# NikNazarov/TorchPIV

Measured on AMD Instinct MI355X. Metric: image-pairs/sec at 4 MP, wind=64 ov=32 2-pass CWS; % HBM roofline, higher is better.
Workload: dtype u32 exact sums + f64 / f32

## Files before the change

torchpiv_amd/csrc/piv_kernels.h:

```cpp
#pragma once
#include <hip/hip_runtime.h>
#include <stdint.h>

namespace tpiv {

enum { MODE_PASS1 = 0, MODE_DWS = 1, MODE_CWS = 2, MODE_CWSF = 3 };

struct PassParams {
    const uint8_t* A;
    const uint8_t* B;
    int batch, H, W;
    int ws, ov, n_rows, n_cols;
    const double* u0;
    const double* v0;
    const double* u2;
    const double* v2;
    const uint8_t* pmask;
    double* u;
    double* v;
    uint8_t* val;
    double* du;
    double* dv;
    double val_ratio;
    int val_win;
    int precision;
    float* dbg_win;
    float* dbg_corr;
    unsigned long long* stamps;
    float* peak_raw;
    unsigned* work_ctr;
    int* slow_list;
    unsigned* slow_count;
    int list_mode;
    uint4* cand;
    int* fb_list;
    unsigned* fb_count;
    float exact_band;
    float exact_band_range;
    hipEvent_t* sub_events;
    unsigned groups_magic, ncols_magic;
    int groups_shift, ncols_shift;
};

constexpr double EXACT_ETA = 6.66;
enum { EXACT_FFT_RADIX2 = 0, EXACT_FFT_MIXED = 1, EXACT_FFT_PLAIN = 2 };
inline double exact_gamma_u(int ws, int kind) {
    double lg = 0.0, rt = 1.0;
    for (int n = 1; n < ws; n *= 2) lg += 1.0;
    while ((rt + 1.0) * (rt + 1.0) <= (double)ws) rt += 1.0;
    rt += 1.0;
    const double f1 = kind == EXACT_FFT_PLAIN ? (ws + 3) * rt : (kind == EXACT_FFT_MIXED ? 64.0 : lg * EXACT_ETA);
    const double i1 = kind == EXACT_FFT_PLAIN ? (double)(ws + 3) : f1;
    return 2.0 * (2.0 * f1 + 1.0) + 5.0 + 2.0 * i1;
}
inline float exact_band_coef(int ws, int kind = EXACT_FFT_RADIX2) {
    return (float)(2.0 * exact_gamma_u(ws, kind) * (1.0 + 1.0 / 16) * 5.9604644775390625e-08);
}
constexpr int EXACT_MAX_SECOND = 3, EXACT_MAX_MIN = 4;

struct PredictParams {
    int batch, mode;
    int nrc, ncc, nrf, ncf;
    const double* Ay;
    const double* Ax;
    const double* u_c;
    const double* v_c;
    const uint8_t* val_c;
    double* T;
    double* u0;
    double* v0;
    double* u2;
    double* v2;
};

struct BandedPredictParams {
    int batch, mode;
    int nrc, ncc, nrf, ncf;
    int KY, KX;
    int nrfp;
    const double* Wy32;
    const int* k0y32;
    const double* Ax32;
    const int* k0x32;
    const double* u_c;
    const double* v_c;
    const uint8_t* val_c;
    double* T1;
    double* u0;
    double* v0;
    double* u2;
    double* v2;
    uint8_t* mask_out;
};

struct PostvalParams {
    double* u;
    double* v;
    const uint8_t* invalid;
    uint8_t* cls;
    int* counts;
    int batch, n_rows, n_cols;
};
hipError_t launch_postval(const PostvalParams& p, hipStream_t stream);
hipError_t launch_postval_compact(const double* u, const double* v, const uint8_t* cls, const int* counts, int batch, int n_rows,
                                  int n_cols, int* offsets, int* ring_rc, double* ring_uv, int* hole_rc, hipStream_t stream);
hipError_t launch_finish_fields(const double* u, const double* v, int batch, int n_rows, int n_cols, double scale, double dt,
                                double* fu, double* fv, hipStream_t stream);
hipError_t launch_ensemble_moments(const double* U, const double* V, int n, long long cells, double* out, hipStream_t stream);

hipError_t launch_bmp_unpack(const uint8_t* raw, const long long* desc, const uint8_t* lut, int n_files, int H, int W,
                             uint8_t* out, hipStream_t stream);

hipError_t launch_xcorr(const PassParams& p, int mode, int n_cu, hipStream_t stream);
constexpr size_t TILE_CTR_BYTES = 8 * 16 * sizeof(unsigned), TILE_SLOW_HDR_BYTES = 256;
#ifndef TPIV_SPLIT64
#define TPIV_SPLIT64 1
#endif
constexpr bool tile_split64(int ws, int mode) { return TPIV_SPLIT64 && ws == 64 && mode == MODE_CWS; }
#ifndef TPIV_OCC64C
#define TPIV_OCC64C 2
#endif
constexpr int tile_occ_c(int ws, int mode) {
    return (ws != 8 && ws != 16 && ws != 32 && ws != 64) ? 0
           : (ws == 16 ? 4 : ((ws == 32 || (ws == 64 && (mode != MODE_CWS || TPIV_OCC64C == 3))) ? 3 : 2));
}
inline int tile_occ(int ws, int mode) { return tile_occ_c(ws, mode); }
#ifdef __HIPCC__
template <int MODE>
__device__ __forceinline__ void pred_half_shift(const PassParams& p, size_t i, double& sx, double& sy) {
    const bool compact = p.pmask != nullptr;
    const double* __restrict__ us = compact ? p.u0 : p.u2;
    const double* __restrict__ vs = compact ? p.v0 : p.v2;
    double u = us[i], v = vs[i];
    if constexpr (MODE == MODE_DWS) {
        const uint8_t* mp = compact ? p.pmask + i : reinterpret_cast<const uint8_t*>(us + i);
        const bool zero = *mp != 0 && compact;
        const double uz = zero ? 0.0 : u, vz = zero ? 0.0 : v;
        sx = compact ? rint(uz / 2) : u;
        sy = compact ? rint(vz / 2) : v;
    } else {
        sx = compact ? u / 2 : u;
        sy = compact ? v / 2 : v;
    }
}
__device__ __forceinline__ void pred_half_shift_cws_f32(const PassParams& p, size_t i, float& vx, float& vy) {
    const bool compact = p.pmask != nullptr;
    const double* __restrict__ us = compact ? p.u0 : p.u2;
    const double* __restrict__ vs = compact ? p.v0 : p.v2;
    const float k = compact ? 0.5f : 1.0f;
    vx = (float)us[i] * k;
    vy = (float)vs[i] * k;
}
__device__ __forceinline__ void pred_fallback(const PassParams& p, size_t i, double& u0, double& v0) {
    const bool compact = p.pmask != nullptr;
    const uint8_t* mp = compact ? p.pmask + i : reinterpret_cast<const uint8_t*>(p.u0 + i);
    const bool zero = *mp != 0 && compact;
    u0 = zero ? 0.0 : p.u0[i];
    v0 = zero ? 0.0 : p.v0[i];
}
#endif

const char* xcorr_kernel_name(int ws, int mode, int precision, char* buf, int len);
size_t peak_raw_bytes(int ws, int batch, int n_windows, int precision, bool force_generic = false);
bool exact_refine_size(int ws);
size_t exact_fallback_count_offset(int batch, int n_windows);
hipError_t launch_peaks_from_maps(const PassParams& p, const float* maps, int n_maps, int planar, hipStream_t stream);
hipError_t launch_predict_mfma(const BandedPredictParams& q, hipStream_t stream);
hipError_t launch_predict(const PredictParams& q, hipStream_t stream);

}
```

torchpiv_amd/csrc/piv_launch.hip:

```cpp
#include <hip/hip_runtime.h>
#include <stdint.h>
#include <stdio.h>
#include <stdlib.h>

#include "piv_kernels.h"

namespace tpiv {

hipError_t launch_xcorr_ws8(const PassParams& p, int mode, int n_cu, hipStream_t stream);
hipError_t launch_xcorr_w8(const PassParams& p, int mode, int n_cu, hipStream_t stream);
hipError_t launch_peak_debug_w8(const PassParams& p, const float* maps, int n_maps, hipStream_t stream);
hipError_t launch_xcorr_ws16(const PassParams& p, int mode, int n_cu, hipStream_t stream);
hipError_t launch_xcorr_ws32(const PassParams& p, int mode, int n_cu, hipStream_t stream);
hipError_t launch_xcorr_ws64(const PassParams& p, int mode, int n_cu, hipStream_t stream);
hipError_t launch_xcorr_big128_pass1(const PassParams& p, int n_cu, hipStream_t stream);
hipError_t launch_peak_debug_ws8(const PassParams& p, const float* maps, int n_maps, int planar, hipStream_t stream);
hipError_t launch_peak_debug_ws16(const PassParams& p, const float* maps, int n_maps, int planar, hipStream_t stream);
hipError_t launch_peak_debug_ws32(const PassParams& p, const float* maps, int n_maps, int planar, hipStream_t stream);
hipError_t launch_peak_debug_ws64(const PassParams& p, const float* maps, int n_maps, int planar, hipStream_t stream);
hipError_t launch_peak_debug_ws128(const PassParams& p, const float* maps, int n_maps, hipStream_t stream);
hipError_t launch_xcorr_generic(const PassParams& p, int mode, int n_cu, void* scratch, hipStream_t stream);
int generic_blocks(int ws, long long items, int n_cu, int elem_bytes);
bool generic_ct_usable(int ws);
int generic_ct_register_size(int ws, int mode);
hipError_t launch_xcorr_f64(const PassParams& p, int n_cu, hipStream_t stream);
hipError_t launch_xcorr_cand_ws8(const PassParams& p, int n_cu, hipStream_t stream);
hipError_t launch_xcorr_cand_ws16(const PassParams& p, int n_cu, hipStream_t stream);
hipError_t launch_xcorr_cand_ws32(const PassParams& p, int n_cu, hipStream_t stream);
hipError_t launch_xcorr_cand_ws64(const PassParams& p, int n_cu, hipStream_t stream);
hipError_t launch_xcorr_cand_ws128(const PassParams& p, int n_cu, hipStream_t stream);
hipError_t launch_exact_refine(const PassParams& p, int n_cu, hipStream_t stream);
bool exact_refine_size(int ws);
hipError_t launch_xcorr_f64_list(const PassParams& p, int n_cu, hipStream_t stream);

__device__ __forceinline__ double nan_to_num_f(double x) {
    if (x != x) return 0.0;
    if (x > 1.7976931348623157e308) return 1.7976931348623157e308;
    if (x < -1.7976931348623157e308) return -1.7976931348623157e308;
    return x;
}

template <bool F64>
__global__ __launch_bounds__(256) void finalize_kernel(PassParams p, int mode) {
    const size_t total = (size_t)p.batch * p.n_rows * p.n_cols;
    const int d_ = p.ws, k_ = (p.ws & 1) ? p.ws - 1 : p.ws;
    for (size_t i = blockIdx.x * (size_t)blockDim.x + threadIdx.x; i < total; i += (size_t)gridDim.x * blockDim.x) {
        double cm, cl, cr, ct, cb, c2;
        int m;
        bool dead;
        if constexpr (F64) {
            const double* __restrict__ rw = reinterpret_cast<const double*>(p.peak_raw) + i * 8;
            cm = rw[0], cl = rw[1], cr = rw[2], ct = rw[3], cb = rw[4], c2 = rw[5];
            m = (int)rw[6];
            dead = rw[7] != 0.0;
        } else {
            const float4* __restrict__ rw = reinterpret_cast<const float4*>(p.peak_raw + i * 8);
            const float4 r0 = rw[0], r1 = rw[1];
            cm = (double)r0.x, cl = (double)r0.y, cr = (double)r0.z, ct = (double)r0.w;
            cb = (double)r1.x, c2 = (double)r1.y;
            m = __float_as_int(r1.z);
            dead = __float_as_int(r1.w) != 0;
        }
        const double lm = log(cm), ll = log(cl), lr = log(cr), lt = log(ct), lb = log(cb);
        const double nom1 = lr - ll;
        const double den1 = 2 * (ll + lr) - 4 * lm;
        const double nom2 = lb - lt;
        const double den2 = 2 * (lb + lt) - 4 * lm;
        double du = (double)(m % k_) + nom1 / den1 - (double)(k_ / 2);
        double dv = (double)(m / d_) + nom2 / den2 - (double)(d_ / 2);
        du = nan_to_num_f(du);
        dv = nan_to_num_f(dv);
        bool invalid = (cm / c2) < p.val_ratio;
        if (mode == MODE_PASS1) {
            if (dead) {
                du = 0.0;
                dv = 0.0;
                invalid = false;
            }
            if (!dead && (m % k_) == k_ / 2 && (m / d_) == d_ / 2 && fabs(du) < 1e-4 && fabs(dv) < 1e-4 && p.A != nullptr) {
                const int pair = (int)(i / ((size_t)p.n_rows * p.n_cols)), win = (int)(i % ((size_t)p.n_rows * p.n_cols));
                const int st = p.ws - p.ov;
                const size_t off = (size_t)pair * p.H * p.W + (size_t)(win / p.n_cols) * st * p.W + (size_t)(win % p.n_cols) * st;
                bool same = true;
                for (int r = 0; r < p.ws && same; ++r) {
                    const uint8_t* __restrict__ ra = p.A + off + (size_t)r * p.W;
                    const uint8_t* __restrict__ rb = p.B + off + (size_t)r * p.W;
                    int c = 0;
                    for (; c + 16 <= p.ws; c += 16) {
                        uint4 va, vb;
                        __builtin_memcpy(&va, ra + c, 16);
                        __builtin_memcpy(&vb, rb + c, 16);
                        same = same && va.x == vb.x && va.y == vb.y && va.z == vb.z && va.w == vb.w;
                    }
                    for (; c < p.ws; ++c) same = same && ra[c] == rb[c];
                }
                if (same) {
                    du = 0.0;
                    dv = 0.0;
                }
            }
            p.u[i] = du;
            p.v[i] = dv;
            p.val[i] = invalid ? 1 : 0;
        } else {
            double u0, v0;
            pred_fallback(p, i, u0, v0);
            double u, v;
            if (mode == MODE_CWSF) {
                u = u0 + du;
                v = v0 + dv;
            } else {
                double sx, sy;
                if (mode == MODE_DWS) pred_half_shift<MODE_DWS>(p, i, sx, sy);
                else pred_half_shift<MODE_CWS>(p, i, sx, sy);
                u = 2 * sx + du;
                v = 2 * sy + dv;
            }
            const bool mask_u = ((du > u0) && (rint(u0) > 0)) || invalid;
            const bool mask_v = ((dv > v0) && (rint(v0) > 0)) || invalid;
            if (mask_u) u = u0;
            if (mask_v) v = v0;
            p.u[i] = u;
            p.v[i] = v;
            p.val[i] = invalid ? 1 : 0;
            if (p.du != nullptr) {
                p.du[i] = du;
                p.dv[i] = dv;
            }
        }
    }
}

static bool tile_size(int ws) { return ws == 8 || ws == 16 || ws == 32 || ws == 64; }
static size_t peak_bytes(int batch, int n_windows, int precision = 0) {
    return (((size_t)batch * n_windows * 8 * (precision ? sizeof(double) : sizeof(float))) + 255) / 256 * 256;
}

hipError_t launch_peaks_from_maps(const PassParams& p, const float* maps, int n_maps, int planar, hipStream_t stream) {
    hipError_t e;
    switch (p.ws) {
        case 8:
            e = planar == 2 ? launch_peak_debug_w8(p, maps, n_maps, stream) : launch_peak_debug_ws8(p, maps, n_maps, planar, stream);
            break;
        case 16: e = launch_peak_debug_ws16(p, maps, n_maps, planar, stream); break;
        case 32: e = launch_peak_debug_ws32(p, maps, n_maps, planar, stream); break;
        case 64: e = launch_peak_debug_ws64(p, maps, n_maps, planar, stream); break;
        case 128: e = launch_peak_debug_ws128(p, maps, n_maps, stream); break;
        default: return hipErrorInvalidValue;
    }
    if (e != hipSuccess) return e;
    hipLaunchKernelGGL(finalize_kernel<false>, dim3((n_maps + 255) / 256), dim3(256), 0, stream, p, (int)MODE_PASS1);
    return hipGetLastError();
}

static constexpr size_t WORK_CTR_BYTES = TILE_CTR_BYTES;
static size_t work_ctr_offset(int batch, int n_windows) { return (peak_bytes(batch, n_windows) + 127) / 128 * 128; }

struct ExactLayout {
    size_t cand, list, count, ctr, scratch, total;
};
static ExactLayout exact_layout(int ws, int batch, int n_windows) {
    auto up = [](size_t b) { return (b + 255) / 256 * 256; };
    ExactLayout l;
    l.cand = peak_bytes(batch, n_windows, 1);
    l.list = l.cand + up((size_t)batch * n_windows * sizeof(uint4));
    l.count = l.list + up((size_t)batch * n_windows * sizeof(int));
    l.ctr = l.count + 256;
    l.scratch = l.ctr + WORK_CTR_BYTES;
    l.total = l.scratch;
    if (!tile_size(ws) && ws != 128)
        l.total += (size_t)generic_blocks(ws, (long long)batch * n_windows, 256, 8) * 2 * ws * ws * 2 * 8;
    return l;
}
static bool exact_size(int ws) { return exact_refine_size(ws); }
size_t exact_fallback_count_offset(int batch, int n_windows) { return exact_layout(64, batch, n_windows).count; }

size_t peak_raw_bytes(int ws, int batch, int n_windows, int precision, bool force_generic) {
    if (precision == 3) {
        if (exact_size(ws) && !force_generic) return exact_layout(ws, batch, n_windows).total;
        precision = 1;
    }
    if (tile_size(ws) && !force_generic) {
        if (precision) return peak_bytes(batch, n_windows, 1);
        return work_ctr_offset(batch, n_windows) + WORK_CTR_BYTES +
               (ws == 64 ? TILE_SLOW_HDR_BYTES + (size_t)batch * n_windows * sizeof(int) : 0);
    }
    const int eb = precision ? 8 : 4;
    return peak_bytes(batch, n_windows, precision) +
           (size_t)generic_blocks(ws, (long long)batch * n_windows, 256, eb) * 2 * ws * ws * 2 * eb;
}

static int pass_precision(int precision, int mode, int ws) {
    if (precision == 2) return mode == MODE_PASS1 ? 1 : 0;
    if (precision == 3) return mode == MODE_PASS1 ? (exact_size(ws) ? 3 : 1) : 0;
    return precision;
}

const char* xcorr_kernel_name(int ws, int mode, int precision, char* buf, int len) {
    precision = pass_precision(precision, mode, ws);
    if (precision == 3 && mode == MODE_PASS1) {
        if (ws == 128) snprintf(buf, len, "xcorr_big128_cand_kernel");
        else if (tile_size(ws)) snprintf(buf, len, "xcorr_tile_cand_kernel<%d>", ws);
        else if (generic_ct_usable(ws)) snprintf(buf, len, "xcorr_generic_ct_kernel<0, %d> (cand)", generic_ct_register_size(ws, mode));
        else snprintf(buf, len, "xcorr_generic_kernel<0, float> (cand)");
    } else if (precision && mode == MODE_PASS1) {
        if (ws == 64 || ws == 128) snprintf(buf, len, "xcorr_f64_split_kernel<%d>", ws);
        else if (tile_size(ws)) snprintf(buf, len, "xcorr_f64_tile_kernel<%d>", ws);
        else snprintf(buf, len, "xcorr_generic_kernel<0, double>");
    } else if (ws == 8) {
        snprintf(buf, len, "xcorr_w8_kernel<%d, %s>", mode, (precision && mode != MODE_PASS1) ? "false" : "true");
    } else if (tile_size(ws)) {
        snprintf(buf, len, "xcorr_tile_kernel<%d, %d, %d, %s>", ws, mode, tile_occ(ws, mode),
                 (precision && mode != MODE_PASS1) ? "false" : "true");
    } else if (ws == 128 && mode == MODE_PASS1) {
        snprintf(buf, len, "xcorr_big128_kernel");
    } else {
        if (generic_ct_usable(ws)) snprintf(buf, len, "xcorr_generic_ct_kernel<%d, %d>", mode, generic_ct_register_size(ws, mode));
        else snprintf(buf, len, "xcorr_generic_kernel<%d, float>", mode);
    }
    if (mode == MODE_CWSF) snprintf(buf, len, generic_ct_usable(ws) ? "xcorr_generic_ct_kernel<3, 0>" : "xcorr_generic_kernel<3, float>");
    return buf;
}

hipError_t launch_xcorr(const PassParams& p_in, int mode, int n_cu, hipStream_t stream) {
    hipError_t e;
    PassParams p = p_in;
    p.precision = pass_precision(p.precision, mode, p.ws);
    const bool f64 = p.precision != 0 && mode == MODE_PASS1;
    auto generic = [&]() {
        if (p.ws < 2 || p.ws > 256) return hipErrorInvalidValue;
        void* scratch = reinterpret_cast<char*>(p.peak_raw) + peak_bytes(p.batch, p.n_rows * p.n_cols, f64 ? 1 : 0);
        PassParams q = p;
        q.precision = f64 ? 1 : 0;
        return launch_xcorr_generic(q, mode, 256, scratch, stream);
    };
    if (mode == MODE_CWSF) {
        e = generic();
    } else if (p.precision == 3) {
        const ExactLayout l = exact_layout(p.ws, p.batch, p.n_rows * p.n_cols);
        char* const base = reinterpret_cast<char*>(p.peak_raw);
        p.cand = reinterpret_cast<uint4*>(base + l.cand);
        p.fb_list = reinterpret_cast<int*>(base + l.list);
        p.fb_count = reinterpret_cast<unsigned*>(base + l.count);
        p.work_ctr = reinterpret_cast<unsigned*>(base + l.ctr);
        static const float band_scale = [] {
            const char* env = getenv("TPIV_EXACT_BAND_SCALE");
            return env ? (float)atof(env) : 1.0f;
        }();
        static const float band_range = [] {
            const char* env = getenv("TPIV_EXACT_BAND_RANGE");
            return env ? (float)atof(env) : 0.0f;
        }();
        const int fft_kind = (tile_size(p.ws) || p.ws == 128) ? EXACT_FFT_RADIX2 : (generic_ct_usable(p.ws) ? EXACT_FFT_MIXED : EXACT_FFT_PLAIN);
        p.exact_band = band_scale * exact_band_coef(p.ws, fft_kind);
        p.exact_band_range = band_range;
        e = hipMemsetAsync(p.fb_count, 0, 256 + WORK_CTR_BYTES, stream);
        if (e != hipSuccess) return e;
        auto mark = [&](int i) {
            if (p.sub_events) (void)hipEventRecord(p.sub_events[i], stream);
        };
        PassParams q = p;
        q.precision = 0;
        void* const gscratch = base + l.scratch;
        switch (p.ws) {
            case 8: e = launch_xcorr_cand_ws8(p, n_cu, stream); break;
            case 16: e = launch_xcorr_cand_ws16(p, n_cu, stream); break;
            case 32: e = launch_xcorr_cand_ws32(p, n_cu, stream); break;
            case 64: e = launch_xcorr_cand_ws64(p, n_cu, stream); break;
            case 128: e = launch_xcorr_cand_ws128(p, n_cu, stream); break;
            default: e = launch_xcorr_generic(q, MODE_PASS1, 256, gscratch, stream); break;
        }
        if (e != hipSuccess) return e;
        mark(0);
        e = launch_exact_refine(p, n_cu, stream);
        if (e != hipSuccess) return e;
        mark(1);
        if (tile_size(p.ws) || p.ws == 128) {
            e = launch_xcorr_f64_list(p, n_cu, stream);
        } else {
            q.precision = 1;
            q.cand = nullptr;
            e = launch_xcorr_generic(q, MODE_PASS1, 256, gscratch, stream);
        }
        mark(2);
    } else if (f64) {
        static const bool gen128 = [] {
            const char* env = getenv("TPIV_F64_GENERIC128");
            return env && env[0] == '1';
        }();
        e = (tile_size(p.ws) || (p.ws == 128 && !gen128)) ? launch_xcorr_f64(p, n_cu, stream) : generic();
    } else if (tile_size(p.ws)) {
        p.work_ctr = reinterpret_cast<unsigned*>(reinterpret_cast<char*>(p.peak_raw) +
                                                 work_ctr_offset(p.batch, p.n_rows * p.n_cols));
        p.list_mode = 0;
        p.slow_list = nullptr;
        p.slow_count = nullptr;
        const bool split = tile_split64(p.ws, mode) && p.precision == 0;
        if (split) {
            p.slow_count = reinterpret_cast<unsigned*>(reinterpret_cast<char*>(p.work_ctr) + WORK_CTR_BYTES);
            p.slow_list = reinterpret_cast<int*>(reinterpret_cast<char*>(p.slow_count) + TILE_SLOW_HDR_BYTES);
        }
        e = hipMemsetAsync(p.work_ctr, 0, WORK_CTR_BYTES + (split ? TILE_SLOW_HDR_BYTES : 0), stream);
        if (e != hipSuccess) return e;
        static const bool w8 = [] {
            const char* env = getenv("TPIV_W8");
            return !(env && env[0] == '0');
        }();
        switch (p.ws) {
            case 8: e = w8 ? launch_xcorr_w8(p, mode, n_cu, stream) : launch_xcorr_ws8(p, mode, n_cu, stream); break;
            case 16: e = launch_xcorr_ws16(p, mode, n_cu, stream); break;
            case 32: e = launch_xcorr_ws32(p, mode, n_cu, stream); break;
            default: e = launch_xcorr_ws64(p, mode, n_cu, stream); break;
        }
    } else if (p.ws == 128 && mode == MODE_PASS1) {
        e = launch_xcorr_big128_pass1(p, n_cu, stream);
    } else {
        e = generic();
    }
    if (e != hipSuccess) return e;
    const size_t total = (size_t)p.batch * p.n_rows * p.n_cols;
    size_t blocks = (total + 255) / 256;
    if (blocks > (size_t)n_cu * 32) blocks = (size_t)n_cu * 32;
    if (f64) hipLaunchKernelGGL(finalize_kernel<true>, dim3((unsigned)blocks), dim3(256), 0, stream, p, mode);
    else hipLaunchKernelGGL(finalize_kernel<false>, dim3((unsigned)blocks), dim3(256), 0, stream, p, mode);
    return hipGetLastError();
}

__global__ void predict_cols_kernel(PredictParams q) {
    const long long total = (long long)q.batch * 3 * q.nrc * q.ncf;
    for (long long i = blockIdx.x * (long long)blockDim.x + threadIdx.x; i < total;
         i += (long long)gridDim.x * blockDim.x) {
        const int cfi = (int)(i % q.ncf);
        const int rc = (int)((i / q.ncf) % q.nrc);
        const int f = (int)((i / ((long long)q.ncf * q.nrc)) % 3);
        const int b = (int)(i / ((long long)q.ncf * q.nrc * 3));
        const double* ax = q.Ax + (size_t)cfi * q.ncc;
        const size_t zoff = ((size_t)b * q.nrc + rc) * q.ncc;
        double acc = 0.0;
        if (f == 2) {
            const uint8_t* z = q.val_c + zoff;
            for (int k = 0; k < q.ncc; ++k) acc += (double)z[k] * ax[k];
        } else {
            const double* z = (f == 0 ? q.u_c : q.v_c) + zoff;
            for (int k = 0; k < q.ncc; ++k) acc += z[k] * ax[k];
        }
        q.T[i] = acc;
    }
}

__global__ void predict_rows_kernel(PredictParams q) {
    const long long total = (long long)q.batch * q.nrf * q.ncf;
    for (long long i = blockIdx.x * (long long)blockDim.x + threadIdx.x; i < total;
         i += (long long)gridDim.x * blockDim.x) {
        const int cfi = (int)(i % q.ncf);
        const int rf = (int)((i / q.ncf) % q.nrf);
        const int b = (int)(i / ((long long)q.ncf * q.nrf));
        const double* ay = q.Ay + (size_t)rf * q.nrc;
        const double* t0 = q.T + ((size_t)b * 3 + 0) * q.nrc * q.ncf + cfi;
        const double* t1 = q.T + ((size_t)b * 3 + 1) * q.nrc * q.ncf + cfi;
        const double* t2 = q.T + ((size_t)b * 3 + 2) * q.nrc * q.ncf + cfi;
        double u0 = 0.0, v0 = 0.0, vm = 0.0;
        for (int k = 0; k < q.nrc; ++k) {
            const double a = ay[k];
            u0 += a * t0[(size_t)k * q.ncf];
            v0 += a * t1[(size_t)k * q.ncf];
            vm += a * t2[(size_t)k * q.ncf];
        }
        const bool val = vm >= 0.5;
        double u2, v2;
        if (q.mode == MODE_CWS) {
            u2 = u0 / 2;
            v2 = v0 / 2;
        }
        if (val) {
            u0 = 0.0;
            v0 = 0.0;
        }
        if (q.mode == MODE_DWS) {
            u2 = rint(u0 / 2);
            v2 = rint(v0 / 2);
        }
        q.u0[i] = u0;
        q.v0[i] = v0;
        q.u2[i] = u2;
        q.v2[i] = v2;
    }
}

hipError_t launch_predict(const PredictParams& q, hipStream_t stream) {
    {
        const long long total = (long long)q.batch * 3 * q.nrc * q.ncf;
        long long blocks = (total + 255) / 256;
        if (blocks > 65536) blocks = 65536;
        hipLaunchKernelGGL(predict_cols_kernel, dim3((unsigned)blocks), dim3(256), 0, stream, q);
        hipError_t e = hipGetLastError();
        if (e != hipSuccess) return e;
    }
    {
        const long long total = (long long)q.batch * q.nrf * q.ncf;
        long long blocks = (total + 255) / 256;
        if (blocks > 65536) blocks = 65536;
        hipLaunchKernelGGL(predict_rows_kernel, dim3((unsigned)blocks), dim3(256), 0, stream, q);
        return hipGetLastError();
    }
}

}
```

torchpiv_amd/csrc/xcorr_exact.hip:

```cpp
#include <hip/hip_runtime.h>
#include <stdint.h>

#include "piv_kernels.h"
#include "xcorr_tile.hpp"

namespace tpiv {

namespace {

template <int W>
struct XGeo {
    static constexpr int NDW = W / 4;
    static constexpr int XP = 2 * NDW + 1;
    static constexpr int GROUP = W < 64 ? W : 64;
    static constexpr int WPW = 64 / GROUP;
    static constexpr int PARTS = W / GROUP;
    static constexpr int WAVES = W == 128 ? 2 : 4;
    static constexpr int WINS = WAVES * WPW / PARTS;
    static constexpr int KD = W * W;
    static constexpr bool COOP = W >= 32;
    static constexpr int P16 = W / 16;
    static constexpr int LW = GROUP * PARTS;
    static constexpr int AP = NDW + 4;
    static_assert(!COOP || (W * AP <= W * XP && (LW * P16) == W * P16), "the hand-over tile lives in the parked rows' memory");
};
constexpr int XCELLS = 5 + EXACT_MAX_SECOND + EXACT_MAX_MIN;

#if defined(__HIP_DEVICE_COMPILE__)
template <int OFF>
__device__ __forceinline__ uint32_t lds_rd32(unsigned addr) {
    uint32_t v;
    asm volatile("ds_read_b32 %0, %1 offset:%2" : "=v"(v) : "v"(addr), "n"(OFF) : "memory");
    return v;
}
__device__ __forceinline__ void lds_landed() { asm volatile("s_waitcnt lgkmcnt(0)" ::: "memory"); }
__device__ __forceinline__ void lds_tie(uint32_t& v) { asm volatile("" : "+v"(v)); }
#else
template <int OFF>
__host__ __device__ inline uint32_t lds_rd32(unsigned) { return 0u; }
__host__ __device__ inline void lds_landed() {}
__host__ __device__ inline void lds_tie(uint32_t&) {}
#endif
template <int N>
__device__ __forceinline__ void read_span(const uint32_t* src, uint32_t (&w)[N]) {
    const unsigned addr = (unsigned)(uintptr_t)src;
    static_for<0, N>([&](auto ic) TPIV_LAMBDA_INLINE { w[decltype(ic)::value] = lds_rd32<4 * decltype(ic)::value>(addr); });
    lds_landed();
    static_for<0, N>([&](auto ic) TPIV_LAMBDA_INLINE { lds_tie(w[decltype(ic)::value]); });
}

__device__ __forceinline__ void list_append(const PassParams& p, bool want, long long it) {
    const unsigned long long mk = __ballot(want);
    if (mk == 0ull) return;
    const int lane = (int)__builtin_amdgcn_mbcnt_hi(~0u, __builtin_amdgcn_mbcnt_lo(~0u, 0u));
    const int leader = (int)__builtin_ctzll(mk);
    unsigned base = 0u;
    if (lane == leader) base = atomicAdd(p.fb_count, (unsigned)__popcll(mk));
    base = (unsigned)__builtin_amdgcn_readlane((int)base, leader);
    if (want) p.fb_list[base + (unsigned)__popcll(mk & ((1ull << lane) - 1ull))] = (int)it;
}

__device__ __forceinline__ void decide_and_store(const PassParams& p, const uint4& rec, int r0, bool go, bool writer, bool have,
                                                 int m, unsigned S, unsigned sa, unsigned sb, double kd, double* out, long long it) {
    auto hi16 = [](unsigned v) TPIV_LAMBDA_INLINE { return (int)(short)(v >> 16); };
    auto umin = [](unsigned x, unsigned y) TPIV_LAMBDA_INLINE { return x < y ? x : y; };
    auto umax = [](unsigned x, unsigned y) TPIV_LAMBDA_INLINE { return x > y ? x : y; };
    auto uadd = [](unsigned x, unsigned y) TPIV_LAMBDA_INLINE { return x + y; };
    constexpr int S0 = 5, N0 = 5 + EXACT_MAX_SECOND;
    S = r0 < XCELLS ? S : 0u;
    const unsigned s_min = grp_reduce<16>((have && r0 >= N0 && r0 < XCELLS) ? S : 0xffffffffu, umin);
    const unsigned s_low = grp_reduce<16>((have && r0 < XCELLS) ? S : 0xffffffffu, umin);
    const unsigned s_top = grp_reduce<16>((have && r0 < N0) ? S : 0u, umax);
    const unsigned s_m = grp_reduce<16>(r0 == 0 ? S : 0u, umax);
    const unsigned s_second = grp_reduce<16>((have && r0 >= S0 && r0 < N0) ? S : 0u, umax);
    const unsigned n_second = grp_reduce<16>((have && r0 >= S0 && r0 < N0) ? 1u : 0u, uadd);
    const bool min_overflow = hi16(rec.w) == -2;
    const bool redo = s_top > s_m || s_low < s_min || s_min == 0xffffffffu || sa == 0u || sb == 0u ||
                      (min_overflow && s_min != 0u);
    list_append(p, go && redo && r0 == 0 && writer, it);
    const double scale = (kd * kd) / ((double)sa * (double)sb);
    const unsigned mine = r0 == 5 ? s_second : S;
    double v = __fma_rn((double)(mine - s_min), scale, 1e-7);
    v = (r0 == 5 && n_second == 0u) ? 0.0 : v;
    v = r0 == 6 ? (double)m : v;
    v = r0 == 7 ? 0.0 : v;
    if (go && !redo && r0 < 8 && writer) out[r0] = v;
}

template <int W>
__global__ __launch_bounds__(64 * XGeo<W>::WAVES) void xcorr_exact_refine_kernel(PassParams p) {
    using G = XGeo<W>;
    constexpr int NDW = G::NDW, XP = G::XP, KD = G::KD;
    __shared__ __attribute__((aligned(16))) uint32_t parked[G::WINS][W * XP];
    __shared__ unsigned joined[2][16];
    const int wave = __builtin_amdgcn_readfirstlane((int)(threadIdx.x >> 6));
    const int lane = (int)(threadIdx.x & 63);
    const int g = lane / G::GROUP, r0 = lane % G::GROUP;
    const int part = G::PARTS == 2 ? wave : 0;
    const int row = r0 + 64 * part;
    const int wslot = G::PARTS == 2 ? 0 : wave * G::WPW + g;
    uint32_t* const rows_b = parked[wslot];
    const int N = p.n_rows * p.n_cols;
    const long long total = (long long)p.batch * N;
    const int xcd = blockIdx.x & 7, slot = blockIdx.x >> 3;
    const long long chunk = (total + 7) / 8;
    const long long in_chunk = (long long)slot * G::WINS + wslot;
    const long long it_raw = (long long)xcd * chunk + in_chunk;
    const bool valid = in_chunk < chunk && it_raw < total;
    const long long it = valid ? it_raw : 0;

    const unsigned itu = (unsigned)it;
    const int pair = (int)(itu / (unsigned)N), win = (int)(itu - (unsigned)pair * (unsigned)N);
    const int st = p.ws - p.ov;
    const size_t off0 = (size_t)pair * p.H * p.W + (size_t)((win / p.n_cols) * st) * p.W + (size_t)(win % p.n_cols) * st;
    uint32_t a[NDW], b[NDW];
    uint32_t ca[G::COOP ? G::P16 : 1][4], cb[G::COOP ? G::P16 : 1][4];
    const int tw = r0 + 64 * part;
    if constexpr (G::COOP) {
#pragma unroll
        for (int k = 0; k < G::P16; ++k) {
            const int ci = tw + G::LW * k, j = ci / G::P16, pt = ci % G::P16;
            const size_t o_ = off0 + (size_t)j * p.W + 16 * pt;
            load_dwords<4>(p.A + o_, ca[k]);
            load_dwords<4>(p.B + o_, cb[k]);
        }
    } else {
        const size_t off = off0 + (size_t)row * p.W;
        load_dwords<NDW>(p.A + off, a);
        load_dwords<NDW>(p.B + off, b);
    }
    const uint4 rec = p.cand[it];
    auto lo16 = [](unsigned v) TPIV_LAMBDA_INLINE { return (int)(short)(v & 0xffffu); };
    auto hi16 = [](unsigned v) TPIV_LAMBDA_INLINE { return (int)(short)(v >> 16); };
    const int m = valid ? lo16(rec.x) : -3;
    double* const out = reinterpret_cast<double*>(p.peak_raw) + (size_t)it * 8;
    const bool writer = part == 0;
    list_append(p, m == -1 && r0 == 0 && writer, it);
    if (m == -2 && r0 < 8 && writer) out[r0] = r0 == 6 ? 0.0 : 1.0;
    const bool go = m >= 0;
    if (__ballot(go) == 0ull) return;

    int q = -1;
    if (go) {
        int left = m + 1, right = m - 1, top = m + W, bot = m - W;
        if (left >= KD - 1) left = m;
        if (right <= 0) right = m;
        if (top >= KD - 1) top = m;
        if (bot <= 0) bot = m;
        q = r0 == 0 ? m : q;
        q = r0 == 1 ? left : q;
        q = r0 == 2 ? right : q;
        q = r0 == 3 ? top : q;
        q = r0 == 4 ? bot : q;
        q = r0 == 5 ? hi16(rec.x) : q;
        q = r0 == 6 ? lo16(rec.y) : q;
        q = r0 == 7 ? hi16(rec.y) : q;
        q = r0 == 8 ? lo16(rec.z) : q;
        q = r0 == 9 ? hi16(rec.z) : q;
        q = r0 == 10 ? lo16(rec.w) : q;
        q = r0 == 11 ? hi16(rec.w) : q;
    }

    unsigned P[16];
#pragma unroll
    for (int k = 0; k < 16; ++k) P[k] = 0u;
    auto lds_sync = [&]() TPIV_LAMBDA_INLINE {
        if constexpr (G::PARTS == 2) __syncthreads();
        else wave_sync();
    };
    if constexpr (G::COOP) {
        uint4* const ta = reinterpret_cast<uint4*>(rows_b);
#pragma unroll
        for (int k = 0; k < G::P16; ++k) {
            const int ci = tw + G::LW * k, j = ci / G::P16, pt = ci % G::P16;
            ta[j * (G::AP / 4) + pt] = make_uint4(ca[k][0], ca[k][1], ca[k][2], ca[k][3]);
        }
        lds_sync();
#pragma unroll
        for (int k = 0; k < NDW / 4; ++k) {
            const uint4 t = ta[row * (G::AP / 4) + k];
            a[4 * k] = t.x, a[4 * k + 1] = t.y, a[4 * k + 2] = t.z, a[4 * k + 3] = t.w;
        }
        lds_sync();
#pragma unroll
        for (int k = 0; k < G::P16; ++k) {
            const int ci = tw + G::LW * k, j = ci / G::P16, pt = ci % G::P16;
#pragma unroll
            for (int c = 0; c < 4; ++c) {
                P[13] = __builtin_amdgcn_sad_u8(cb[k][c], 0u, P[13]);
                rows_b[j * XP + 4 * pt + c] = cb[k][c];
                rows_b[j * XP + NDW + 4 * pt + c] = cb[k][c];
            }
        }
#pragma unroll
        for (int i = 0; i < NDW; ++i) P[12] = __builtin_amdgcn_sad_u8(a[i], 0u, P[12]);
    } else {
#pragma unroll
        for (int i = 0; i < NDW; ++i) {
            P[12] = __builtin_amdgcn_sad_u8(a[i], 0u, P[12]);
            P[13] = __builtin_amdgcn_sad_u8(b[i], 0u, P[13]);
            rows_b[row * XP + i] = b[i];
            rows_b[row * XP + NDW + i] = b[i];
        }
    }
    lds_sync();

    static_for<0, XCELLS>([&](auto cc) TPIV_LAMBDA_INLINE {
        constexpr int c = decltype(cc)::value;
        int qc = __builtin_amdgcn_readlane(q, c);
        bool any = qc >= 0;
        static_for<1, G::WPW>([&](auto wc) TPIV_LAMBDA_INLINE {
            constexpr int k = decltype(wc)::value;
            const int qk = __builtin_amdgcn_readlane(q, k * G::GROUP + c);
            any = any || qk >= 0;
            qc = g == k ? qk : qc;
        });
        if (any) {
            const bool on = qc >= 0;
            const int qq = on ? qc : 0;
            const int dy = qq / W - W / 2, dx = qq % W - W / 2;
            const int brow = (row + dy) & (W - 1), bx = dx & (W - 1);
            const uint32_t* src = rows_b + brow * XP + (bx >> 2);
            const unsigned sh = (unsigned)(bx & 3);
            uint32_t w[NDW + 1];
            read_span<NDW + 1>(src, w);
            unsigned acc = 0;
#pragma unroll
            for (int i = 0; i < NDW; ++i) acc = __builtin_amdgcn_udot4(a[i], __builtin_amdgcn_alignbyte(w[i + 1], w[i], sh), acc, false);
            P[c] = on ? acc : 0u;
        }
    });
    unsigned T[4];
    {
        const bool odd = lane & 1, hi = lane & 2;
        unsigned Q[8];
#pragma unroll
        for (int j = 0; j < 8; ++j) {
            const unsigned keep = odd ? P[2 * j + 1] : P[2 * j], send = odd ? P[2 * j] : P[2 * j + 1];
            Q[j] = keep + (unsigned)dpp_i<DPP_XOR1>((int)send);
        }
#pragma unroll
        for (int j = 0; j < 4; ++j) {
            const unsigned keep = hi ? Q[2 * j + 1] : Q[2 * j], send = hi ? Q[2 * j] : Q[2 * j + 1];
            unsigned t = keep + (unsigned)dpp_i<DPP_XOR2>((int)send);
            t += (unsigned)dpp_i<0x128>((int)t);
            t += (unsigned)dpp_i<0x124>((int)t);
            if constexpr (G::GROUP >= 32) {
                auto r = __builtin_amdgcn_permlane16_swap(t, t, false, false);
                t = r[0] + r[1];
            }
            if constexpr (G::GROUP >= 64) {
                auto r = __builtin_amdgcn_permlane32_swap(t, t, false, false);
                t = r[0] + r[1];
            }
            T[j] = t;
        }
    }
    unsigned S = r0 < 4 ? T[0] : (r0 < 8 ? T[1] : (r0 < 12 ? T[2] : T[3]));
    if constexpr (G::PARTS == 2) {
        if (lane < 16) joined[wave][lane] = S;
        __syncthreads();
        S = lane < 16 ? joined[0][lane] + joined[1][lane] : 0u;
        T[3] = S;
    }
    unsigned sa, sb;
    {
        const unsigned t3 = (r0 & 12) == 12 ? T[3] : 0u;
        unsigned rowsum = t3;
        rowsum += (unsigned)dpp_i<0x128>((int)rowsum);
        rowsum += (unsigned)dpp_i<0x124>((int)rowsum);
        sa = (unsigned)dpp_i<0x00>((int)rowsum);
        sb = (unsigned)dpp_i<0x55>((int)rowsum);
    }
    S = r0 < XCELLS ? S : 0u;

    decide_and_store(p, rec, r0, go, writer, q >= 0, m, S, sa, sb, (double)KD, out, it);
}

template <int W>
struct SGeo {
    static constexpr int NDW = W / 4, XP = 2 * NDW + 1, STRIP = (W * XP) | 1, KD = W * W;
};
template <int W>
struct SBlock {
    static constexpr int SW = W == 8 ? 4 : 1;
};
template <int W>
__global__ __launch_bounds__(64 * SBlock<W>::SW) void xcorr_exact_refine_small_kernel(PassParams p) {
    using G = SGeo<W>;
    constexpr int NDW = G::NDW, XP = G::XP, KD = G::KD, SW = SBlock<W>::SW, NT = 64 * SW;
    __shared__ uint32_t strips[NT * G::STRIP];
    __shared__ unsigned blk_n, blk_base;
    const int lane = (int)threadIdx.x;
    uint32_t* const mine = strips + lane * G::STRIP;
    if (SW > 1 && lane == 0) blk_n = 0u;
    const int N = p.n_rows * p.n_cols;
    const long long total = (long long)p.batch * N;
    const int xcd = blockIdx.x & 7, slot = blockIdx.x >> 3;
    const long long chunk = (total + 7) / 8;
    const long long in_chunk = (long long)slot * NT + lane;
    const long long it_raw = (long long)xcd * chunk + in_chunk;
    const bool valid = in_chunk < chunk && it_raw < total;
    const long long it = valid ? it_raw : 0;
    const unsigned itu = (unsigned)it;
    const int pair = (int)(itu / (unsigned)N), win = (int)(itu - (unsigned)pair * (unsigned)N);
    const int st = p.ws - p.ov;
    const size_t off = (size_t)pair * p.H * p.W + (size_t)((win / p.n_cols) * st) * p.W + (size_t)(win % p.n_cols) * st;
    const uint4 rec = p.cand[it];
    uint32_t a[W][NDW];
    unsigned sa = 0u, sb = 0u;
#pragma unroll
    for (int y = 0; y < W; ++y) {
        uint32_t b[NDW];
        load_dwords<NDW>(p.A + off + (size_t)y * p.W, a[y]);
        load_dwords<NDW>(p.B + off + (size_t)y * p.W, b);
#pragma unroll
        for (int i = 0; i < NDW; ++i) {
            sa = __builtin_amdgcn_sad_u8(a[y][i], 0u, sa);
            sb = __builtin_amdgcn_sad_u8(b[i], 0u, sb);
            mine[y * XP + i] = b[i];
            mine[y * XP + NDW + i] = b[i];
        }
    }
    auto lo16 = [](unsigned v) TPIV_LAMBDA_INLINE { return (int)(short)(v & 0xffffu); };
    auto hi16 = [](unsigned v) TPIV_LAMBDA_INLINE { return (int)(short)(v >> 16); };
    const int m = valid ? lo16(rec.x) : -3;
    double* const out = reinterpret_cast<double*>(p.peak_raw) + (size_t)it * 8;
    if (m == -2) {
#pragma unroll
        for (int r = 0; r < 8; ++r) out[r] = r == 6 ? 0.0 : 1.0;
    }
    const bool go = m >= 0;
    bool redo = false;
    if (__ballot(go) != 0ull) {
    int q[XCELLS];
    {
        int left = m + 1, right = m - 1, top = m + W, bot = m - W;
        if (left >= KD - 1) left = m;
        if (right <= 0) right = m;
        if (top >= KD - 1) top = m;
        if (bot <= 0) bot = m;
        q[0] = m, q[1] = left, q[2] = right, q[3] = top, q[4] = bot;
        q[5] = hi16(rec.x), q[6] = lo16(rec.y), q[7] = hi16(rec.y);
        q[8] = lo16(rec.z), q[9] = hi16(rec.z), q[10] = lo16(rec.w), q[11] = hi16(rec.w);
    }
    wave_sync();
    unsigned S[XCELLS];
    static_for<0, XCELLS>([&](auto cc) TPIV_LAMBDA_INLINE {
        constexpr int c = decltype(cc)::value;
        const bool on = go && q[c] >= 0;
        unsigned acc = 0u;
        if (__ballot(on) != 0ull) {
            const int qq = on ? q[c] : 0;
            const int dy = qq / W - W / 2, bx = (qq % W - W / 2) & (W - 1);
            const unsigned sh = (unsigned)(bx & 3);
            const uint32_t* const src = mine + (bx >> 2);
#pragma unroll
            for (int y = 0; y < W; ++y) {
                const uint32_t* rowp = src + ((y + dy) & (W - 1)) * XP;
                uint32_t w[NDW + 1];
#pragma unroll
                for (int i = 0; i <= NDW; ++i) w[i] = rowp[i];
#pragma unroll
                for (int i = 0; i < NDW; ++i) acc = __builtin_amdgcn_udot4(a[y][i], __builtin_amdgcn_alignbyte(w[i + 1], w[i], sh), acc, false);
            }
        }
        S[c] = on ? acc : 0u;
    });
    constexpr int S0 = 5, N0 = 5 + EXACT_MAX_SECOND;
    unsigned s_min = 0xffffffffu, s_low = 0xffffffffu, s_top = 0u, s_second = 0u, n_second = 0u;
#pragma unroll
    for (int c = 0; c < XCELLS; ++c) {
        const bool have = q[c] >= 0;
        if (c >= N0) s_min = (have && S[c] < s_min) ? S[c] : s_min;
        s_low = (have && S[c] < s_low) ? S[c] : s_low;
        if (c < N0) s_top = (have && S[c] > s_top) ? S[c] : s_top;
        if (c >= S0 && c < N0) {
            s_second = (have && S[c] > s_second) ? S[c] : s_second;
            n_second += have ? 1u : 0u;
        }
    }
    const unsigned s_m = S[0];
    const bool min_overflow = hi16(rec.w) == -2;
    redo = s_top > s_m || s_low < s_min || s_min == 0xffffffffu || sa == 0u || sb == 0u || (min_overflow && s_min != 0u);
    if (go && !redo) {
        const double scale = ((double)KD * (double)KD) / ((double)sa * (double)sb);
#pragma unroll
        for (int r = 0; r < 5; ++r) out[r] = __fma_rn((double)(S[r] - s_min), scale, 1e-7);
        out[5] = n_second == 0u ? 0.0 : __fma_rn((double)(s_second - s_min), scale, 1e-7);
        out[6] = (double)m;
        out[7] = 0.0;
    }
    }
    const bool want = m == -1 || (go && redo);
    if constexpr (SW == 1) {
        list_append(p, want, it);
    } else {
        const unsigned long long mk = __ballot(want);
        const int wl = lane & 63;
        unsigned wbase = 0u;
        __syncthreads();
        if (mk != 0ull && wl == 0) wbase = atomicAdd(&blk_n, (unsigned)__popcll(mk));
        wbase = (unsigned)__builtin_amdgcn_readfirstlane((int)wbase);
        __syncthreads();
        if (lane == 0 && blk_n != 0u) blk_base = atomicAdd(p.fb_count, blk_n);
        __syncthreads();
        if (want) p.fb_list[blk_base + wbase + (unsigned)__popcll(mk & ((1ull << wl) - 1ull))] = (int)it;
    }
}

template <int G>
__global__ __launch_bounds__(64) void xcorr_exact_refine_any_kernel(PassParams p, int ndw, int xp) {
    extern __shared__ uint32_t any_smem[];
    constexpr int LPW = 64 / G, SL = LPW / 16;
    const int W = p.ws, KD = W * W;
    const int lane = (int)threadIdx.x;
    const int g = lane / LPW, c = lane & 15, k = (lane % LPW) >> 4;
    const int N = p.n_rows * p.n_cols;
    const long long total = (long long)p.batch * N;
    const int xcd = blockIdx.x & 7, slot = blockIdx.x >> 3;
    const long long chunk = (total + 7) / 8;
    const int st = p.ws - p.ov;
    const bool dwords = (W & 3) == 0;
    const float rcp_ndw = 1.0f / (float)ndw;

    unsigned sa_w[G], sb_w[G];
    long long it_w[G];
    bool valid_w[G];
    static_for<0, G>([&](auto gc) TPIV_LAMBDA_INLINE {
        constexpr int gi = decltype(gc)::value;
        const long long in_chunk = (long long)slot * G + gi;
        const long long it_raw = (long long)xcd * chunk + in_chunk;
        valid_w[gi] = in_chunk < chunk && it_raw < total;
        it_w[gi] = valid_w[gi] ? it_raw : 0;
        const unsigned itu = (unsigned)it_w[gi];
        const int pair = (int)(itu / (unsigned)N), win = (int)(itu - (unsigned)pair * (unsigned)N);
        const size_t off = (size_t)pair * p.H * p.W + (size_t)((win / p.n_cols) * st) * p.W + (size_t)(win % p.n_cols) * st;
        const uint8_t* __restrict__ A0 = p.A + off;
        const uint8_t* __restrict__ B0 = p.B + off;
        uint32_t* const ag = any_smem + gi * W * ndw;
        uint32_t* const bg = any_smem + G * W * ndw + gi * W * xp;
        uint8_t* const bgb = reinterpret_cast<uint8_t*>(bg);
        unsigned pa = 0u, pb = 0u;
        for (int idx = lane; idx < W * ndw; idx += 64) {
            const int row = (int)(((float)idx + 0.5f) * rcp_ndw), i = idx - row * ndw;
            const uint8_t* ra = A0 + (size_t)row * p.W + 4 * i;
            const uint8_t* rb = B0 + (size_t)row * p.W + 4 * i;
            uint32_t da = 0u, db = 0u;
            const int nb = W - 4 * i < 4 ? W - 4 * i : 4;
            if (nb == 4) {
                __builtin_memcpy(&da, ra, 4);
                __builtin_memcpy(&db, rb, 4);
            } else {
                for (int t = 0; t < nb; ++t) {
                    da |= (uint32_t)ra[t] << (8 * t);
                    db |= (uint32_t)rb[t] << (8 * t);
                }
            }
            ag[row * ndw + i] = da;
            pa = __builtin_amdgcn_sad_u8(da, 0u, pa);
            pb = __builtin_amdgcn_sad_u8(db, 0u, pb);
            if (dwords) {
                bg[row * xp + i] = db;
                bg[row * xp + ndw + i] = db;
            } else {
                for (int t = 0; t < nb; ++t) {
                    const uint8_t v = (uint8_t)(db >> (8 * t));
                    bgb[row * xp * 4 + 4 * i + t] = v;
                    bgb[row * xp * 4 + W + 4 * i + t] = v;
                }
            }
        }
        auto uadd = [](unsigned x, unsigned y) TPIV_LAMBDA_INLINE { return x + y; };
        sa_w[gi] = grp_reduce<64>(pa, uadd);
        sb_w[gi] = grp_reduce<64>(pb, uadd);
    });
    wave_sync();

    long long it = it_w[0];
    bool valid = valid_w[0];
    unsigned sa = sa_w[0], sb = sb_w[0];
    static_for<1, G>([&](auto gc) TPIV_LAMBDA_INLINE {
        constexpr int gi = decltype(gc)::value;
        it = g == gi ? it_w[gi] : it;
        valid = g == gi ? valid_w[gi] : valid;
        sa = g == gi ? sa_w[gi] : sa;
        sb = g == gi ? sb_w[gi] : sb;
    });
    const uint4 rec = p.cand[it];
    auto lo16 = [](unsigned v) TPIV_LAMBDA_INLINE { return (int)(short)(v & 0xffffu); };
    auto hi16 = [](unsigned v) TPIV_LAMBDA_INLINE { return (int)(short)(v >> 16); };
    const int m = valid ? lo16(rec.x) : -3;
    double* const out = reinterpret_cast<double*>(p.peak_raw) + (size_t)it * 8;
    const bool writer = k == 0;
    list_append(p, m == -1 && c == 0 && writer, it);
    if (m == -2 && c < 8 && writer) out[c] = c == 6 ? 0.0 : 1.0;
    const bool go = m >= 0;
    if (__ballot(go) == 0ull) return;
    int q = -1;
    if (go) {
        int left = m + 1, right = m - 1, top = m + W, bot = m - W;
        if (left >= KD - 1) left = m;
        if (right <= 0) right = m;
        if (top >= KD - 1) top = m;
        if (bot <= 0) bot = m;
        q = c == 0 ? m : q;
        q = c == 1 ? left : q;
        q = c == 2 ? right : q;
        q = c == 3 ? top : q;
        q = c == 4 ? bot : q;
        q = c == 5 ? hi16(rec.x) : q;
        q = c == 6 ? lo16(rec.y) : q;
        q = c == 7 ? hi16(rec.y) : q;
        q = c == 8 ? lo16(rec.z) : q;
        q = c == 9 ? hi16(rec.z) : q;
        q = c == 10 ? lo16(rec.w) : q;
        q = c == 11 ? hi16(rec.w) : q;
    }
    unsigned S = 0u;
    {
        const bool on = q >= 0;
        const int qq = on ? q : 0;
        const int qy = qq / W, qx = qq - qy * W;
        int dy = qy - W / 2, bx = qx - W / 2;
        bx += bx < 0 ? W : 0;
        const unsigned sh = (unsigned)(bx & 3);
        const uint32_t* const ag = any_smem + g * W * ndw;
        const uint32_t* const bg = any_smem + G * W * ndw + g * W * xp + (bx >> 2);
        for (int y = k; y < W; y += SL) {
            int by = y + dy;
            by += by < 0 ? W : 0;
            by -= by >= W ? W : 0;
            const uint32_t* ar = ag + y * ndw;
            const uint32_t* br = bg + by * xp;
            uint32_t prev = br[0];
            for (int i = 0; i < ndw; ++i) {
                const uint32_t nxt = br[i + 1];
                S = __builtin_amdgcn_udot4(ar[i], __builtin_amdgcn_alignbyte(nxt, prev, sh), S, false);
                prev = nxt;
            }
        }
        S = on ? S : 0u;
    }
    if constexpr (SL == 4) {
        auto r = __builtin_amdgcn_permlane16_swap(S, S, false, false);
        S = r[0] + r[1];
        auto r2 = __builtin_amdgcn_permlane32_swap(S, S, false, false);
        S = r2[0] + r2[1];
    }
    decide_and_store(p, rec, c, go, writer, q >= 0, m, S, sa, sb, (double)KD, out, it);
}

}

template <int W>
static hipError_t launch_refine(const PassParams& p, hipStream_t stream) {
    using G = XGeo<W>;
    const long long total = (long long)p.batch * p.n_rows * p.n_cols;
    const long long chunk = (total + 7) / 8;
    const long long slots = (chunk + G::WINS - 1) / G::WINS;
    hipLaunchKernelGGL((xcorr_exact_refine_kernel<W>), dim3((unsigned)(slots * 8)), dim3(64 * G::WAVES), 0, stream, p);
    return hipGetLastError();
}

template <int W>
static hipError_t launch_refine_small(const PassParams& p, hipStream_t stream) {
    const long long total = (long long)p.batch * p.n_rows * p.n_cols;
    const long long chunk = (total + 7) / 8;
    constexpr int NT = 64 * SBlock<W>::SW;
    const long long slots = (chunk + NT - 1) / NT;
    hipLaunchKernelGGL((xcorr_exact_refine_small_kernel<W>), dim3((unsigned)(slots * 8)), dim3(NT), 0, stream, p);
    return hipGetLastError();
}

template <int G>
static hipError_t launch_refine_any(const PassParams& p, hipStream_t stream) {
    const int W = p.ws, ndw = (W + 3) / 4;
    const int xp = ((2 * W + 6 + 3) / 4) | 1;
    const long long total = (long long)p.batch * p.n_rows * p.n_cols;
    const long long chunk = (total + 7) / 8;
    const long long slots = (chunk + G - 1) / G;
    const size_t smem = (size_t)G * W * (ndw + xp) * sizeof(uint32_t);
    if (smem > 64 * 1024) return hipErrorInvalidValue;
    hipLaunchKernelGGL((xcorr_exact_refine_any_kernel<G>), dim3((unsigned)(slots * 8)), dim3(64), smem, stream, p, ndw, xp);
    return hipGetLastError();
}

bool exact_refine_size(int ws) { return ws >= 8 && ws <= 128 && (ws & 1) == 0; }

hipError_t launch_exact_refine(const PassParams& p, int n_cu, hipStream_t stream) {
    const long long total = (long long)p.batch * p.n_rows * p.n_cols;
    if (total <= 0 || total >= (1ll << 31) || p.cand == nullptr || p.fb_list == nullptr || p.fb_count == nullptr ||
        !exact_refine_size(p.ws))
        return hipErrorInvalidValue;
    static const bool small_on = [] { const char* e = getenv("TPIV_REFINE_SMALL"); return !(e && e[0] == '0'); }();
    switch (p.ws) {
        case 8:
            if (small_on) return launch_refine_small<8>(p, stream);
            return launch_refine_any<4>(p, stream);
        case 16: return small_on ? launch_refine_small<16>(p, stream) : launch_refine<16>(p, stream);
        case 32: return launch_refine<32>(p, stream);
        case 64: return launch_refine<64>(p, stream);
        case 128: return launch_refine<128>(p, stream);
        default: return p.ws <= 32 ? launch_refine_any<4>(p, stream) : launch_refine_any<1>(p, stream);
    }
}

}
```

torchpiv_amd/csrc/xcorr_tile.hpp:

```cpp
#pragma once
#include <hip/hip_runtime.h>
#include <stdint.h>
#include <stdlib.h>

#include "fft_inreg.hpp"
#include "piv_kernels.h"

namespace tpiv {

template <int WS, bool PLANAR_ = false>
struct TileGeo {
    static constexpr int WPW = 64 / WS;
    static constexpr int TS = WS > 32 ? 32 : WS;
    static constexpr int PITCH = TS + 1;
    static constexpr int NT = 64 / TS;
    static constexpr int TILE = TS * PITCH;
    static constexpr bool PLANAR = PLANAR_;
    static constexpr int HROWS = WS / 2 + 1;
    static constexpr int HTILE = HROWS * PITCH;
    static constexpr int LDS_FLOATS = NT * TILE * (PLANAR ? 1 : 2);
    static constexpr int MAP_PITCH = WS + 1;
    static constexpr int NDW = WS / 4;
};

template <int CTRL>
__device__ __forceinline__ int dpp_i(int v) {
    return __builtin_amdgcn_update_dpp(0, v, CTRL, 0xF, 0xF, true);
}
template <int CTRL>
__device__ __forceinline__ float dpp_f(float v) {
    return __int_as_float(dpp_i<CTRL>(__float_as_int(v)));
}
constexpr int DPP_XOR1 = 0xB1;
constexpr int DPP_XOR2 = 0x4E;
constexpr int DPP_HALF_MIRROR = 0x141;
constexpr int DPP_ROW_MIRROR = 0x140;

template <int HALF>
__device__ __forceinline__ void partner2(int a, int& pa) {
    if constexpr (HALF == 1) pa = dpp_i<DPP_XOR1>(a);
    else if constexpr (HALF == 2) pa = dpp_i<DPP_XOR2>(a);
    else if constexpr (HALF == 4) pa = dpp_i<DPP_HALF_MIRROR>(a);
    else if constexpr (HALF == 8) pa = dpp_i<DPP_ROW_MIRROR>(a);
}

template <int WS, typename T, typename OP>
__device__ __forceinline__ T grp_reduce(T v, OP op) {
    static_assert(sizeof(T) == 4 || sizeof(T) == 8, "one or two dwords");
    constexpr int NW = sizeof(T) / 4;
    union U {
        T t;
        int w[NW];
    };
    static_for<0, 4>([&](auto sc) TPIV_LAMBDA_INLINE {
        constexpr int half = 1 << decltype(sc)::value;
        if constexpr (half < WS) {
            U a, b;
            a.t = v;
#pragma unroll
            for (int q = 0; q < NW; ++q) partner2<half>(a.w[q], b.w[q]);
            v = op(v, b.t);
        }
    });
    if constexpr (WS >= 32) {
        U a, x, y;
        a.t = v;
#pragma unroll
        for (int q = 0; q < NW; ++q) {
            auto r = __builtin_amdgcn_permlane16_swap((unsigned)a.w[q], (unsigned)a.w[q], false, false);
            x.w[q] = (int)r[0];
            y.w[q] = (int)r[1];
        }
        v = op(x.t, y.t);
    }
    if constexpr (WS >= 64) {
        U a, x, y;
        a.t = v;
#pragma unroll
        for (int q = 0; q < NW; ++q) {
            auto r = __builtin_amdgcn_permlane32_swap((unsigned)a.w[q], (unsigned)a.w[q], false, false);
            x.w[q] = (int)r[0];
            y.w[q] = (int)r[1];
        }
        v = op(x.t, y.t);
    }
    return v;
}

template <int WS>
__device__ __forceinline__ float grp_sum(float v) {
    return grp_reduce<WS>(v, [](float a, float b) TPIV_LAMBDA_INLINE { return a + b; });
}

template <int WS>
__device__ __forceinline__ float grp_min(float v) {
    return grp_reduce<WS>(v, [](float a, float b) TPIV_LAMBDA_INLINE { return fminf(a, b); });
}

__device__ __forceinline__ float fetch_clamped_t(const uint8_t* __restrict__ f, long long q, int HW) {
    q = q < 0 ? 0 : (q > (long long)(HW - 1) ? (long long)(HW - 1) : q);
    return (float)f[q];
}

__device__ __forceinline__ int f2i_sat_t(float v) {
    v = fminf(fmaxf(v, -1073741824.f), 1073741824.f);
    return (int)v;
}

template <int K, int N>
__device__ __forceinline__ float byte_f(const uint32_t (&d)[N]) {
    return (float)((d[K >> 2] >> (8 * (K & 3))) & 0xffu);
}

#ifndef TPIV_SDWA_LERP
#define TPIV_SDWA_LERP 0
#endif
constexpr float SDWA_UP = 0x1p125f, SDWA_DN = 0x1p-24f, SDWA_INV = 0x1p24f;
template <int K, int N>
__device__ __forceinline__ float byte_d(const uint32_t (&d)[N]) {
    return __uint_as_float((d[K >> 2] >> (8 * (K & 3))) & 0xffu);
}

template <int N>
__device__ __forceinline__ void load_dwords(const uint8_t* __restrict__ p, uint32_t (&d)[N]) {
    __builtin_memcpy(&d[0], p, 4 * N);
}

__device__ __forceinline__ float bilerp_ref(float f11, float f21, float f12, float f22, float wx_up,
                                            float wx_dn, float wy_up, float wy_dn, bool degenerate) {
#pragma clang fp contract(off)
    float r = (f11 * wx_up) * wy_up;
    r = r + (f21 * wx_dn) * wy_up;
    r = r + (f12 * wx_up) * wy_dn;
    r = r + (f22 * wx_dn) * wy_dn;
    return degenerate ? f11 : r;
}

__device__ __forceinline__ float bilerp_ref_m(float f11, float f21, float f12, float f22, float wx_up,
                                              float wx_dn, float wy_up, float wy_dn, unsigned degenerate_mask) {
#pragma clang fp contract(off)
    float r = (f11 * wx_up) * wy_up;
    r = r + (f21 * wx_dn) * wy_up;
    r = r + (f12 * wx_up) * wy_dn;
    r = r + (f22 * wx_dn) * wy_dn;
    const unsigned bits = (degenerate_mask & __float_as_uint(f11)) | (~degenerate_mask & __float_as_uint(r));
    return __uint_as_float(bits);
}

#ifdef TPIV_STAMPS
#define TPIV_STAMP_DECL unsigned long long st_acc[16] = {}; unsigned long long st_prev = 0; unsigned st_iter = 0; \
    unsigned long long st_t0 = __builtin_amdgcn_s_memtime(), st_r0 = __builtin_amdgcn_s_memrealtime();
#define TPIV_STAMP_START                                                                  \
    do {                                                                                  \
        __builtin_amdgcn_sched_barrier(0);                                                \
        asm volatile("s_memtime %0\n\ts_waitcnt lgkmcnt(0)" : "=s"(st_prev)::"memory");    \
        __builtin_amdgcn_sched_barrier(0);                                                \
    } while (0)
#define TPIV_STAMP(i)                                                                     \
    do {                                                                                  \
        unsigned long long st_t;                                                          \
        __builtin_amdgcn_sched_barrier(0);                                                \
        asm volatile("s_memtime %0\n\ts_waitcnt lgkmcnt(0)" : "=s"(st_t)::"memory");       \
        __builtin_amdgcn_sched_barrier(0);                                                \
        st_acc[i] += st_t - st_prev;                                                      \
        st_prev = st_t;                                                                   \
    } while (0)
#define TPIV_STAMP_FLUSH(pp)                                                              \
    do {                                                                                  \
        if ((pp).stamps != nullptr && threadIdx.x == 0) {                                 \
            for (int q_ = 0; q_ < 16; ++q_) atomicAdd(&(pp).stamps[q_], st_acc[q_]);      \
            atomicAdd(&(pp).stamps[16], (unsigned long long)st_iter);                     \
            atomicAdd(&(pp).stamps[17], __builtin_amdgcn_s_memtime() - st_t0);            \
            atomicAdd(&(pp).stamps[18], __builtin_amdgcn_s_memrealtime() - st_r0);        \
        }                                                                                 \
    } while (0)
#else
#define TPIV_STAMP_DECL
#define TPIV_STAMP_START
#define TPIV_STAMP(i)
#define TPIV_STAMP_FLUSH(pp)
#endif

__device__ __forceinline__ int fast_div(int n, unsigned magic, int shift) {
    return (int)(((unsigned long long)(unsigned)n * magic) >> shift);
}
inline void fast_div_setup(unsigned d, unsigned& magic, int& shift) {
    int s_ = 0;
    while ((1ull << s_) < d) ++s_;
    shift = 31 + s_;
    magic = (unsigned)(((1ull << shift) + d - 1) / d);
}

__device__ __forceinline__ int fresh_lane() {
    int l = (int)__builtin_amdgcn_mbcnt_hi(~0u, __builtin_amdgcn_mbcnt_lo(~0u, 0u));
    asm volatile("" : "+v"(l));
    return l;
}

__device__ __forceinline__ void wave_sync() {
    __builtin_amdgcn_fence(__ATOMIC_ACQ_REL, "wavefront");
    __builtin_amdgcn_wave_barrier();
}

template <int WS, bool DIGITREV, bool PLANAR>
__device__ __forceinline__ void transpose_tile(cf (&a)[WS], float* lds, int lane) {
    using G = TileGeo<WS, PLANAR>;
    constexpr int P = G::PITCH;
    cf* tile = reinterpret_cast<cf*>(lds);
    if constexpr (PLANAR && WS > 32) {
        static_for<0, 32>([&](auto kc) TPIV_LAMBDA_INLINE {
            constexpr int k = decltype(kc)::value;
            constexpr int lo = DIGITREV ? FFT_POS<k, WS> : k;
            constexpr int hi = DIGITREV ? FFT_POS<k + 32, WS> : k + 32;
            auto rx = __builtin_amdgcn_permlane32_swap(__float_as_uint(a[lo].x), __float_as_uint(a[hi].x),
                                                       false, false);
            auto ry = __builtin_amdgcn_permlane32_swap(__float_as_uint(a[lo].y), __float_as_uint(a[hi].y),
                                                       false, false);
            a[lo].x = __uint_as_float(rx[0]);
            a[hi].x = __uint_as_float(rx[1]);
            a[lo].y = __uint_as_float(ry[0]);
            a[hi].y = __uint_as_float(ry[1]);
        });
        float* t = lds + (lane >> 5) * G::TILE;
        const int i = lane & 31;
        auto plane = [&](auto comp) TPIV_LAMBDA_INLINE {
            constexpr bool Y = decltype(comp)::value;
            float lowhalf[32];
            wave_sync();
            static_for<0, 32>([&](auto kc) TPIV_LAMBDA_INLINE {
                constexpr int k = decltype(kc)::value;
                constexpr int src = DIGITREV ? FFT_POS<k, WS> : k;
                t[i * P + k] = Y ? a[src].y : a[src].x;
            });
            wave_sync();
#pragma unroll
            for (int r = 0; r < 32; ++r) lowhalf[r] = t[r * P + i];
            wave_sync();
            static_for<0, 32>([&](auto kc) TPIV_LAMBDA_INLINE {
                constexpr int k = decltype(kc)::value;
                constexpr int src = DIGITREV ? FFT_POS<k + 32, WS> : k + 32;
                t[i * P + k] = Y ? a[src].y : a[src].x;
            });
            wave_sync();
#pragma unroll
            for (int r = 0; r < 32; ++r) {
                if constexpr (Y) {
                    a[32 + r].y = t[r * P + i];
                    a[r].y = lowhalf[r];
                } else {
                    a[32 + r].x = t[r * P + i];
                    a[r].x = lowhalf[r];
                }
            }
        };
        plane(std::false_type{});
        plane(std::true_type{});
    } else if constexpr (PLANAR) {
        float* t = lds + (lane / WS) * G::TILE;
        const int i = lane % WS;
        wave_sync();
        static_for<0, WS>([&](auto kc) TPIV_LAMBDA_INLINE {
            constexpr int k = decltype(kc)::value;
            constexpr int src = DIGITREV ? FFT_POS<k, WS> : k;
            t[i * P + k] = a[src].x;
        });
        wave_sync();
#pragma unroll
        for (int r = 0; r < WS; ++r) a[r].x = t[r * P + i];
        wave_sync();
        static_for<0, WS>([&](auto kc) TPIV_LAMBDA_INLINE {
            constexpr int k = decltype(kc)::value;
            constexpr int src = DIGITREV ? FFT_POS<k, WS> : k;
            t[i * P + k] = a[src].y;
        });
        wave_sync();
#pragma unroll
        for (int r = 0; r < WS; ++r) a[r].y = t[r * P + i];
    } else if constexpr (WS <= 32) {
        cf* t = tile + (lane / WS) * G::TILE;
        const int i = lane % WS;
        wave_sync();
        static_for<0, WS>([&](auto kc) TPIV_LAMBDA_INLINE {
            constexpr int k = decltype(kc)::value;
            constexpr int src = DIGITREV ? FFT_POS<k, WS> : k;
            t[i * P + k] = a[src];
        });
        wave_sync();
#pragma unroll
        for (int r = 0; r < WS; ++r) a[r] = t[r * P + i];
    } else {
        static_for<0, 32>([&](auto kc) TPIV_LAMBDA_INLINE {
            constexpr int k = decltype(kc)::value;
            constexpr int lo = DIGITREV ? FFT_POS<k, WS> : k;
            constexpr int hi = DIGITREV ? FFT_POS<k + 32, WS> : k + 32;
            auto rx = __builtin_amdgcn_permlane32_swap(__float_as_uint(a[lo].x), __float_as_uint(a[hi].x),
                                                       false, false);
            auto ry = __builtin_amdgcn_permlane32_swap(__float_as_uint(a[lo].y), __float_as_uint(a[hi].y),
                                                       false, false);
            a[lo].x = __uint_as_float(rx[0]);
            a[hi].x = __uint_as_float(rx[1]);
            a[lo].y = __uint_as_float(ry[0]);
            a[hi].y = __uint_as_float(ry[1]);
        });
        cf* t = tile + (lane >> 5) * G::TILE;
        const int i = lane & 31;
        cf lowhalf[32];
        wave_sync();
        static_for<0, 32>([&](auto kc) TPIV_LAMBDA_INLINE {
            constexpr int k = decltype(kc)::value;
            constexpr int src = DIGITREV ? FFT_POS<k, WS> : k;
            t[i * P + k] = a[src];
        });
        wave_sync();
#pragma unroll
        for (int r = 0; r < 32; ++r) lowhalf[r] = t[r * P + i];
        wave_sync();
        static_for<0, 32>([&](auto kc) TPIV_LAMBDA_INLINE {
            constexpr int k = decltype(kc)::value;
            constexpr int src = DIGITREV ? FFT_POS<k + 32, WS> : k + 32;
            t[i * P + k] = a[src];
        });
        wave_sync();
#pragma unroll
        for (int r = 0; r < 32; ++r) a[32 + r] = t[r * P + i];
#pragma unroll
        for (int r = 0; r < 32; ++r) a[r] = lowhalf[r];
    }
}

template <int WS, bool PLANAR>
__device__ __forceinline__ void transpose_half(const cf (&a)[WS], cf (&g)[WS / 2 + 1], float* lds, int lane) {
    static_assert(WS <= 32 || WS == 64, "one tile per window");
    using G = TileGeo<WS, PLANAR>;
    constexpr int P = G::PITCH, M = WS / 2;
    const int i = lane % WS;
    if constexpr (WS == 64) {
        constexpr int Q = M + 1;
        static_assert(WS * Q * (PLANAR ? 1 : 2) <= G::LDS_FLOATS, "half-spectrum plane fits the tile");
        cf b[WS];
        static_for<0, WS>([&](auto kc) TPIV_LAMBDA_INLINE {
            constexpr int k = decltype(kc)::value;
            b[k] = a[FFT_POS<k, WS>];
            asm volatile("" : "+v"(b[k].x), "+v"(b[k].y));
        });
        wave_sync();
        if constexpr (!PLANAR) {
            cf* t = reinterpret_cast<cf*>(lds);
            if (i <= M) {
                static_for<0, WS>([&](auto kc) TPIV_LAMBDA_INLINE {
                    constexpr int k = decltype(kc)::value;
                    t[k * Q + i] = b[k];
                });
            }
            wave_sync();
#pragma unroll
            for (int r = 0; r <= M; ++r) g[r] = t[i * Q + r];
        } else {
        if (i <= M) {
            static_for<0, WS>([&](auto kc) TPIV_LAMBDA_INLINE {
                constexpr int k = decltype(kc)::value;
                lds[k * Q + i] = b[k].x;
            });
        }
        wave_sync();
#pragma unroll
        for (int r = 0; r <= M; ++r) g[r].x = lds[i * Q + r];
        wave_sync();
        if (i <= M) {
            static_for<0, WS>([&](auto kc) TPIV_LAMBDA_INLINE {
                constexpr int k = decltype(kc)::value;
                lds[k * Q + i] = b[k].y;
            });
        }
        wave_sync();
#pragma unroll
        for (int r = 0; r <= M; ++r) g[r].y = lds[i * Q + r];
        }
    } else if constexpr (PLANAR) {
        float* t = lds + (lane / WS) * G::HTILE;
        wave_sync();
        if (i <= M) {
            static_for<0, WS>([&](auto kc) TPIV_LAMBDA_INLINE {
                constexpr int k = decltype(kc)::value;
                t[i * P + k] = a[FFT_POS<k, WS>].x;
            });
        }
        wave_sync();
#pragma unroll
        for (int r = 0; r <= M; ++r) g[r].x = t[r * P + i];
        wave_sync();
        if (i <= M) {
            static_for<0, WS>([&](auto kc) TPIV_LAMBDA_INLINE {
                constexpr int k = decltype(kc)::value;
                t[i * P + k] = a[FFT_POS<k, WS>].y;
            });
        }
        wave_sync();
#pragma unroll
        for (int r = 0; r <= M; ++r) g[r].y = t[r * P + i];
    } else {
        cf* t = reinterpret_cast<cf*>(lds) + (lane / WS) * G::HTILE;
        wave_sync();
        if (i <= M) {
            static_for<0, WS>([&](auto kc) TPIV_LAMBDA_INLINE {
                constexpr int k = decltype(kc)::value;
                t[i * P + k] = a[FFT_POS<k, WS>];
            });
        }
        wave_sync();
#pragma unroll
        for (int r = 0; r <= M; ++r) g[r] = t[r * P + i];
    }
}

struct ItemGeom {
    int pair, win, y0, x0;
    int active;
    size_t fidx;
};

#ifndef TPIV_COOP1
#define TPIV_COOP1 0
#endif
template <int WS>
struct Coop1 {
    static constexpr bool ON = TPIV_COOP1 && (WS == 64 || WS == 32);
    static constexpr int P16 = WS / 16;
    static constexpr int PITCH4 = WS / 16 + 1;
};
template <int WS, int MODE>
struct RawRows;
template <int WS>
struct RawRows<WS, MODE_PASS1> {
    uint32_t a[WS / 4], b[WS / 4];
};
template <int WS>
struct RawRows<WS, MODE_DWS> {
    uint32_t a[WS / 4], b[WS / 4];
    long long qa, qb;
    int reg;
    int cls;
    int fix;
};
template <int WS>
struct CoopGeo {
#ifndef TPIV_COOP
#define TPIV_COOP 1
#endif
    static constexpr bool ON = TPIV_COOP && (WS == 16 || WS == 32 || WS == 64);
    static constexpr int NROW = WS + 1;
    static constexpr int RPG = (WS + 1 + 15) / 16;
    static constexpr int LOADED = 16 * RPG;
    static constexpr int T = NROW * RPG;
    static constexpr int NCH = (T + WS - 1) / WS;
    static constexpr int PITCH4 = RPG | 1;
    static constexpr int PATCH4 = NROW * PITCH4;
    static constexpr int BLOCK4 = (2 * PATCH4 + 15) / 16 * 16;
    static constexpr int FLOATS = (64 / WS) * BLOCK4 * 4;
    static constexpr int LDS_FLOATS = FLOATS + (64 / WS) * (WS + 1) * 4;
    static_assert(!ON || RPG <= PITCH4, "patch row pitch");
    __device__ static __forceinline__ void chunk(int ci, int& j, int& part) {
        if constexpr (RPG == 2) {
            j = ci >> 1;
            part = ci & 1;
        } else if constexpr (RPG == 3) {
            j = (ci * 171) >> 9;
            part = ci - 3 * j;
        } else {
            static_assert(RPG == 5, "chunks per row");
            j = (ci * 205) >> 10;
            part = ci - 5 * j;
        }
    }
};
template <int WS>
struct CoopOff {
    int o[CoopGeo<WS>::ON ? CoopGeo<WS>::NCH : 1];
    __device__ __forceinline__ void init(int r, int W) {
        if constexpr (CoopGeo<WS>::ON) {
#pragma unroll
            for (int k = 0; k < CoopGeo<WS>::NCH; ++k) {
                int j, part;
                CoopGeo<WS>::chunk(r + WS * k, j, part);
                o[k] = r + WS * k < CoopGeo<WS>::T ? j * W + 16 * part : 0;
            }
        }
    }
};
template <int WS>
struct RawRows<WS, MODE_CWS> {
    static constexpr int NB = WS / 4 + 1;
    uint32_t a0[CoopGeo<WS>::ON ? 1 : NB], a1[CoopGeo<WS>::ON ? 1 : NB], b0[CoopGeo<WS>::ON ? 1 : NB], b1[CoopGeo<WS>::ON ? 1 : NB];
    uint32_t ca[CoopGeo<WS>::ON ? CoopGeo<WS>::NCH : 1][4], cb[CoopGeo<WS>::ON ? CoopGeo<WS>::NCH : 1][4];
    int reg;
    int cls;
    int fix;
};

struct CwsRow {
    float wya_up, wya_dn, wyb_up, wyb_dn;
    int dya, uya, dyb, uyb;
    int ydeg_a, ydeg_b;
};
__device__ __forceinline__ CwsRow cws_row(int gy, float vy) {
    CwsRow c;
    const float gyf = (float)gy;
    const float nya = gyf - vy, nyb = gyf + vy;
    const float uya_f = ceilf(nya), dya_f = floorf(nya);
    const float uyb_f = ceilf(nyb), dyb_f = floorf(nyb);
    c.uya = f2i_sat_t(uya_f);
    c.dya = f2i_sat_t(dya_f);
    c.uyb = f2i_sat_t(uyb_f);
    c.dyb = f2i_sat_t(dyb_f);
    c.wya_up = uya_f - nya;
    c.wya_dn = nya - dya_f;
    c.wyb_up = uyb_f - nyb;
    c.wyb_dn = nyb - dyb_f;
    c.ydeg_a = c.uya == c.dya;
    c.ydeg_b = c.uyb == c.dyb;
    return c;
}

__device__ __forceinline__ int classify_row(long long q, int used, int loaded, int HW, long long& qload) {
    const long long lim = (long long)HW - loaded;
    if (q >= 0 && q <= lim) {
        qload = q;
        return 0;
    }
    if (q + used - 1 <= 0) {
        qload = 0;
        return 1;
    }
    if (q >= (long long)HW - 1) {
        qload = lim;
        return 2;
    }
    qload = 0;
    return 3;
}

__device__ __forceinline__ int clamp_i(int v, int lo, int hi) { return v < lo ? lo : (v > hi ? hi : v); }

__device__ __forceinline__ int classify_row32(int q, int used, int loaded, int HW, int& qload) {
    const int lim = HW - loaded;
    const bool inside = (unsigned)q <= (unsigned)lim;
    const bool before = q + used - 1 <= 0;
    const bool behind = q >= HW - 1;
    qload = inside ? q : (behind && !before ? lim : 0);
    return inside ? 0 : (before ? 1 : (behind ? 2 : 3));
}

template <int N>
__device__ __forceinline__ void fix_row(uint32_t (&d)[N], int cls) {
    const uint32_t px = (cls == 1 ? (d[0] & 0xffu) : (d[N - 1] >> 24)) * 0x01010101u;
#pragma unroll
    for (int i = 0; i < N; ++i) d[i] = cls != 0 ? px : d[i];
}
template <int N>
__device__ __forceinline__ void fix_row(uint32_t (&d)[N], int cls, uint32_t last) {
    const uint32_t px = (cls == 1 ? (d[0] & 0xffu) : (last >> 24)) * 0x01010101u;
#pragma unroll
    for (int i = 0; i < N; ++i) d[i] = cls != 0 ? px : d[i];
}

template <int WS, int MODE, bool FAST = false>
__device__ __forceinline__ void issue_rows(const PassParams& p, const ItemGeom& g, int r, float vx, float vy,
                                           RawRows<WS, MODE>& raw, const CoopOff<WS>& coff) {
    const int HW = p.H * p.W;
    const uint8_t* __restrict__ fa = p.A + (size_t)g.pair * HW;
    const uint8_t* __restrict__ fb = p.B + (size_t)g.pair * HW;
    const long long base = (long long)(g.y0 + r) * p.W + g.x0;
    if constexpr (MODE == MODE_PASS1) {
        if constexpr (Coop1<WS>::ON) {
            using C1 = Coop1<WS>;
            const unsigned o0 = (unsigned)(g.y0 * p.W + g.x0);
#pragma unroll
            for (int k = 0; k < C1::P16; ++k) {
                const int ci = r + WS * k, j = ci / C1::P16, part = ci % C1::P16;
                const unsigned o_ = o0 + (unsigned)(j * p.W + 16 * part);
                load_dwords<4>(fa + o_, *reinterpret_cast<uint32_t(*)[4]>(&raw.a[4 * k]));
                load_dwords<4>(fb + o_, *reinterpret_cast<uint32_t(*)[4]>(&raw.b[4 * k]));
            }
        } else {
#ifdef TPIV_EXP_P1LOADS
            load_dwords<4 * TPIV_EXP_P1LOADS>(fa + base, *reinterpret_cast<uint32_t(*)[4 * TPIV_EXP_P1LOADS]>(&raw.a[0]));
            load_dwords<4 * TPIV_EXP_P1LOADS>(fb + base, *reinterpret_cast<uint32_t(*)[4 * TPIV_EXP_P1LOADS]>(&raw.b[0]));
#pragma unroll
            for (int k = 4 * TPIV_EXP_P1LOADS; k < WS / 4; ++k) {
                raw.a[k] = 0x11213141u * (unsigned)(r + 1 + k);
                raw.b[k] = 0x31112141u * (unsigned)(r + 3 + k);
            }
#else
            load_dwords<WS / 4>(fa + base, raw.a);
            load_dwords<WS / 4>(fb + base, raw.b);
#endif
        }
    } else if constexpr (MODE == MODE_DWS) {
        const long long sh = (long long)vy * p.W + (long long)vx;
        raw.qa = base - sh;
        raw.qb = base + sh;
        long long la, lb;
        const int ca = classify_row(raw.qa, WS, WS, HW, la), cb = classify_row(raw.qb, WS, WS, HW, lb);
        raw.reg = __all(ca != 3 && cb != 3) ? 1 : 0;
        raw.cls = ca | (cb << 2);
        raw.fix = (raw.reg && __any(raw.cls != 0)) ? 1 : 0;
        load_dwords<WS / 4>(fa + (raw.reg ? la : base), raw.a);
        load_dwords<WS / 4>(fb + (raw.reg ? lb : base), raw.b);
    } else {
        constexpr int NB = WS / 4 + 1;
        const CwsRow c = cws_row(g.y0 + r, vy);
        const float fvx = floorf(vx);
        const int W_ = p.W;
        const int ivx = clamp_i(f2i_sat_t(fvx), -W_, W_);
        const int rlo = -8, rhi = p.H + 7;
        const int dya = clamp_i(c.dya, rlo, rhi), uya = clamp_i(c.uya, rlo, rhi);
        const int dyb = clamp_i(c.dyb, rlo, rhi), uyb = clamp_i(c.uyb, rlo, rhi);
        const int xa = g.x0 - ivx - 1, xb = g.x0 + ivx;
        const int qa0 = dya * W_ + xa, qa1 = uya * W_ + xa;
        const int qb0 = dyb * W_ + xb, qb1 = uyb * W_ + xb;
        using CG = CoopGeo<WS>;
        constexpr int LOADED = CG::ON ? CG::LOADED : 4 * NB;
        const float gxr = (float)(g.x0 + r);
        const float nxa_r = gxr - vx, nxb_r = gxr + vx;
        const float fxa_r = floorf(nxa_r), fxb_r = floorf(nxb_r);
        const bool col_ok = fxa_r == (float)(g.x0 + r - ivx - 1) && fxb_r == (float)(g.x0 + r + ivx) &&
                            fxa_r != nxa_r && fxb_r != nxb_r;
        bool reg = col_ok && fabsf(vx) < (float)p.W && !(FAST && (c.ydeg_a | c.ydeg_b));
        int la0 = 0, la1 = 0, lb0 = 0, lb1 = 0, cls = 0;
        auto classify_own = [&]() TPIV_LAMBDA_INLINE {
            const int c0 = classify_row32(qa0, WS + 1, LOADED, HW, la0), c1 = classify_row32(qa1, WS + 1, LOADED, HW, la1);
            const int c2 = classify_row32(qb0, WS + 1, LOADED, HW, lb0), c3 = classify_row32(qb1, WS + 1, LOADED, HW, lb1);
            reg = reg && c0 != 3 && c1 != 3 && c2 != 3 && c3 != 3;
            cls = c0 | (c1 << 2) | (c2 << 4) | (c3 << 6);
        };
        if constexpr (CG::ON) {
            const float gy0f = (float)g.y0;
            const int base_a = clamp_i(f2i_sat_t(floorf(gy0f - vy)), rlo, rhi);
            const int base_b = clamp_i(f2i_sat_t(floorf(gy0f + vy)), rlo, rhi);
            reg = reg && (unsigned)(dya - base_a) <= (unsigned)WS && (unsigned)(uya - base_a) <= (unsigned)WS &&
                  (unsigned)(dyb - base_b) <= (unsigned)WS && (unsigned)(uyb - base_b) <= (unsigned)WS;
            const bool inside = base_a >= 0 && base_a + WS < p.H && base_b >= 0 && base_b + WS < p.H &&
                                xa >= 0 && xa + LOADED <= W_ && xb >= 0 && xb + LOADED <= W_;
            const bool all_in = __all(inside);
            if (!all_in) classify_own();
            raw.reg = __all(reg) ? 1 : 0;
            raw.cls = cls;
            raw.fix = (raw.reg && __any(raw.cls != 0)) ? 1 : 0;
            unsigned oa[CG::NCH], ob[CG::NCH];
            if (all_in) {
                const int qa_o = base_a * W_ + xa, qb_o = base_b * W_ + xb;
#pragma unroll
                for (int k = 0; k < CG::NCH; ++k) {
                    oa[k] = (unsigned)(qa_o + coff.o[k]);
                    ob[k] = (unsigned)(qb_o + coff.o[k]);
                }
            } else {
#pragma unroll
                for (int k = 0; k < CG::NCH; ++k) {
                    const int ci = r + WS * k;
                    int j, part;
                    CG::chunk(ci, j, part);
                    int qa_l, qb_l;
                    const int ra = clamp_i(base_a + j, rlo, rhi), rb = clamp_i(base_b + j, rlo, rhi);
                    classify_row32(ra * W_ + xa, WS + 1, LOADED, HW, qa_l);
                    classify_row32(rb * W_ + xb, WS + 1, LOADED, HW, qb_l);
                    const bool live = ci < CG::T;
                    oa[k] = live ? (unsigned)(qa_l + 16 * part) : 0u;
                    ob[k] = live ? (unsigned)(qb_l + 16 * part) : 0u;
                }
            }
#pragma unroll
            for (int k = 0; k < CG::NCH; ++k) {
                load_dwords<4>(fa + oa[k], raw.ca[k]);
                load_dwords<4>(fb + ob[k], raw.cb[k]);
            }
        } else {
        classify_own();
        raw.reg = __all(reg) ? 1 : 0;
        raw.cls = cls;
        raw.fix = (raw.reg && __any(raw.cls != 0)) ? 1 : 0;
        const int lim = HW - 4 * NB;
        const int base32 = (g.y0 + r) * W_ + g.x0;
        const int safe = base32 < lim ? base32 : lim;
        load_dwords<NB>(fa + (unsigned)(raw.reg ? la0 : safe), raw.a0);
        load_dwords<NB>(fa + (unsigned)(raw.reg ? la1 : safe), raw.a1);
        load_dwords<NB>(fb + (unsigned)(raw.reg ? lb0 : safe), raw.b0);
        load_dwords<NB>(fb + (unsigned)(raw.reg ? lb1 : safe), raw.b1);
        }
    }
}

__device__ __forceinline__ uint32_t read_unit_x(const uint4* src) {
    uint4 t = *src;
    asm volatile("" : "+v"(t.x), "+v"(t.y), "+v"(t.z), "+v"(t.w));
    return t.x;
}

struct RowSquares {
    unsigned aa, bb;
};
template <int WS, int MODE, int RBH = 1, bool FAST = false, bool SQ = false, int PATH = 0>
__device__ __forceinline__ void convert_rows(const PassParams& p, const ItemGeom& g, int r, int lane, float vx,
                                             float vy, RawRows<WS, MODE>& raw, cf (&x)[WS], float& sa,
                                             float& sb, float* lds, RowSquares* sq = nullptr) {
    const int HW = p.H * p.W;
    const uint8_t* __restrict__ fa = p.A + (size_t)g.pair * HW;
    const uint8_t* __restrict__ fb = p.B + (size_t)g.pair * HW;
    static constexpr int RBL = WS / RBH;
    float* rowbuf = lds + lane * (RBL + 1);
    static constexpr int UNR_DWS = WS <= 16 ? 1 : 4, UNR_CWS = WS <= 16 ? 1 : 2;
    if constexpr (MODE == MODE_PASS1) {
        if constexpr (Coop1<WS>::ON) {
            using C1 = Coop1<WS>;
            uint4* const t4 = reinterpret_cast<uint4*>(lds) + (lane / WS) * (WS * C1::PITCH4);
            auto hand_over = [&](uint32_t (&d)[WS / 4]) TPIV_LAMBDA_INLINE {
                wave_sync();
#pragma unroll
                for (int k = 0; k < C1::P16; ++k) {
                    const int ci = r + WS * k, j = ci / C1::P16, part = ci % C1::P16;
                    t4[j * C1::PITCH4 + part] = make_uint4(d[4 * k], d[4 * k + 1], d[4 * k + 2], d[4 * k + 3]);
                }
                wave_sync();
#pragma unroll
                for (int k = 0; k < C1::P16; ++k) {
                    const uint4 v = t4[r * C1::PITCH4 + k];
                    d[4 * k] = v.x, d[4 * k + 1] = v.y, d[4 * k + 2] = v.z, d[4 * k + 3] = v.w;
                }
            };
            hand_over(raw.a);
            hand_over(raw.b);
            wave_sync();
        }
        unsigned ia = 0, ib = 0;
#pragma unroll
        for (int q = 0; q < WS / 4; ++q) {
            ia = __builtin_amdgcn_sad_u8(raw.a[q], 0u, ia);
            ib = __builtin_amdgcn_sad_u8(raw.b[q], 0u, ib);
        }
        sa = (float)ia;
        sb = (float)ib;
        if constexpr (SQ) {
            unsigned iaa = 0, ibb = 0;
#pragma unroll
            for (int q = 0; q < WS / 4; ++q) {
                iaa = __builtin_amdgcn_udot4(raw.a[q], raw.a[q], iaa, false);
                ibb = __builtin_amdgcn_udot4(raw.b[q], raw.b[q], ibb, false);
            }
            sq->aa = iaa;
            sq->bb = ibb;
        }
        static_for<0, WS>([&](auto kc) TPIV_LAMBDA_INLINE {
            constexpr int k = decltype(kc)::value;
            x[k].x = byte_f<k, WS / 4>(raw.a);
            x[k].y = byte_f<k, WS / 4>(raw.b);
        });
    } else if constexpr (MODE == MODE_DWS) {
        if (raw.reg) {
            if (raw.fix) {
                fix_row(raw.a, raw.cls & 3);
                fix_row(raw.b, (raw.cls >> 2) & 3);
            }
            static_for<0, WS>([&](auto kc) TPIV_LAMBDA_INLINE {
                constexpr int k = decltype(kc)::value;
                x[k].x = byte_f<k, WS / 4>(raw.a);
                x[k].y = byte_f<k, WS / 4>(raw.b);
            });
        } else {
            wave_sync();
            static_for<0, RBH>([&](auto hc) TPIV_LAMBDA_INLINE {
                constexpr int k0 = decltype(hc)::value * RBL;
#pragma unroll UNR_DWS
                for (int k = 0; k < RBL; ++k) rowbuf[k] = fetch_clamped_t(fa, raw.qa + k0 + k, HW);
#pragma unroll
                for (int k = 0; k < RBL; ++k) x[k0 + k].x = rowbuf[k];
#pragma unroll UNR_DWS
                for (int k = 0; k < RBL; ++k) rowbuf[k] = fetch_clamped_t(fb, raw.qb + k0 + k, HW);
#pragma unroll
                for (int k = 0; k < RBL; ++k) x[k0 + k].y = rowbuf[k];
            });
            wave_sync();
        }
        sa = 0.f;
        sb = 0.f;
        if constexpr (!FAST) {
#pragma unroll
            for (int k = 0; k < WS; ++k) {
                sa += x[k].x;
                sb += x[k].y;
            }
        }
    } else {
        constexpr int NB = WS / 4 + 1;
        const CwsRow c = cws_row(g.y0 + r, vy);
        const float gx0f = (float)g.x0;
        using CG = CoopGeo<WS>;
        if (PATH == 1 || raw.reg) {
            uint32_t ra0[NB], ra1[NB], rb0[NB], rb1[NB];
            const uint4 *lz0 = nullptr, *lz1 = nullptr, *lz2 = nullptr, *lz3 = nullptr;
            if constexpr (CG::ON) {
                uint4* pl = reinterpret_cast<uint4*>(lds);
                const int w_ = lane / WS;
                uint4* pa = pl + w_ * CG::BLOCK4;
                uint4* pb = pa + CG::PATCH4;
                wave_sync();
#pragma unroll
                for (int k = 0; k < CG::NCH; ++k) {
                    const int ci = r + WS * k;
                    int j, part;
                    CG::chunk(ci, j, part);
                    if (ci < CG::T) {
                        pa[j * CG::PITCH4 + part] = make_uint4(raw.ca[k][0], raw.ca[k][1], raw.ca[k][2], raw.ca[k][3]);
                        pb[j * CG::PITCH4 + part] = make_uint4(raw.cb[k][0], raw.cb[k][1], raw.cb[k][2], raw.cb[k][3]);
                    }
                }
                wave_sync();
                const int rlo = -8, rhi = p.H + 7;
                const float gy0f = (float)g.y0;
                const int base_a = clamp_i(f2i_sat_t(floorf(gy0f - vy)), rlo, rhi);
                const int base_b = clamp_i(f2i_sat_t(floorf(gy0f + vy)), rlo, rhi);
                const uint4* s0 = pa + (clamp_i(c.dya, rlo, rhi) - base_a) * CG::PITCH4;
                const uint4* s1 = pa + (clamp_i(c.uya, rlo, rhi) - base_a) * CG::PITCH4;
                const uint4* s2 = pb + (clamp_i(c.dyb, rlo, rhi) - base_b) * CG::PITCH4;
                const uint4* s3 = pb + (clamp_i(c.uyb, rlo, rhi) - base_b) * CG::PITCH4;
                auto fetch = [&](const uint4* src, uint32_t (&d)[NB]) TPIV_LAMBDA_INLINE {
#pragma unroll
                    for (int q = 0; q < NB / 4; ++q) {
                        const uint4 t = src[q];
                        d[4 * q] = t.x, d[4 * q + 1] = t.y, d[4 * q + 2] = t.z, d[4 * q + 3] = t.w;
                    }
                    static_assert(CG::RPG * 4 >= NB, "patch rows hold the whole 16-byte unit of the last dword");
                    d[NB - 1] = read_unit_x(src + NB / 4);
                };
                if (raw.fix) {
                    constexpr int LAST = CG::LOADED / 4 - 1;
                    auto fix_lds = [&](const uint4* src, int cls) TPIV_LAMBDA_INLINE {
                        if (cls != 0) {
                            const uint32_t* sw = reinterpret_cast<const uint32_t*>(src);
                            const uint32_t px = (cls == 1 ? (sw[0] & 0xffu) : (sw[LAST] >> 24)) * 0x01010101u;
                            uint4* dst = const_cast<uint4*>(src);
#pragma unroll
                            for (int q = 0; q < CG::RPG; ++q) dst[q] = make_uint4(px, px, px, px);
                        }
                    };
                    fix_lds(s0, raw.cls & 3);
                    fix_lds(s1, (raw.cls >> 2) & 3);
                    fix_lds(s2, (raw.cls >> 4) & 3);
                    fix_lds(s3, (raw.cls >> 6) & 3);
                    wave_sync();
                }
                constexpr bool LAZY = FAST && WS == 64;
                if constexpr (LAZY) {
                    lz0 = s0, lz1 = s1, lz2 = s2, lz3 = s3;
                } else {
                    fetch(s0, ra0);
                    fetch(s1, ra1);
                    fetch(s2, rb0);
                    fetch(s3, rb1);
                }
            } else {
#pragma unroll
                for (int q = 0; q < NB; ++q) ra0[q] = raw.a0[q], ra1[q] = raw.a1[q], rb0[q] = raw.b0[q], rb1[q] = raw.b1[q];
                if (raw.fix) {
                    fix_row(ra0, raw.cls & 3);
                    fix_row(ra1, (raw.cls >> 2) & 3);
                    fix_row(rb0, (raw.cls >> 4) & 3);
                    fix_row(rb1, (raw.cls >> 6) & 3);
                }
            }
            float4* wbuf = reinterpret_cast<float4*>(lds + (CG::ON ? CG::FLOATS : 0)) + (lane / WS) * (WS + 1);
            {
                const float gxf = gx0f + (float)r;
                const float nxa = gxf - vx, nxb = gxf + vx;
                const float uxa_f = ceilf(nxa), dxa_f = floorf(nxa);
                const float uxb_f = ceilf(nxb), dxb_f = floorf(nxb);
                wave_sync();
                wbuf[r] = make_float4(uxa_f - nxa, nxa - dxa_f, uxb_f - nxb, nxb - dxb_f);
                wave_sync();
            }
            if constexpr (FAST) {
                constexpr bool LAZY = CG::ON && WS == 64;
                auto pull = [&](auto qc) TPIV_LAMBDA_INLINE {
                    constexpr int q = decltype(qc)::value;
                    auto one = [&](const uint4* src, uint32_t (&d)[NB]) TPIV_LAMBDA_INLINE {
                        if constexpr (4 * q + 3 < NB) {
                            const uint4 t = src[q];
                            d[4 * q] = t.x, d[4 * q + 1] = t.y, d[4 * q + 2] = t.z, d[4 * q + 3] = t.w;
                        } else {
                            d[NB - 1] = read_unit_x(src + NB / 4);
                        }
                    };
                    one(lz0, ra0), one(lz1, ra1), one(lz2, rb0), one(lz3, rb1);
                };
                if constexpr (LAZY) {
                    pull(std::integral_constant<int, 0>{});
                    pull(std::integral_constant<int, 1>{});
                }
                constexpr bool SD = TPIV_SDWA_LERP != 0;
                const float wau = SD ? c.wya_up * SDWA_UP : c.wya_up, wad = SD ? c.wya_dn * SDWA_DN : c.wya_dn;
                const float wbu = SD ? c.wyb_up * SDWA_UP : c.wyb_up, wbd = SD ? c.wyb_dn * SDWA_DN : c.wyb_dn;
                auto row_lerp = [&](auto kc, const uint32_t (&r0_)[NB], const uint32_t (&r1_)[NB], float wu_, float wd_) TPIV_LAMBDA_INLINE {
                    constexpr int k = decltype(kc)::value;
                    if constexpr (SD) return fmaf(byte_f<k, NB>(r1_), wd_, byte_d<k, NB>(r0_) * wu_);
                    else return fmaf(byte_f<k, NB>(r1_), wd_, byte_f<k, NB>(r0_) * wu_);
                };
                float va = row_lerp(std::integral_constant<int, 0>{}, ra0, ra1, wau, wad);
                float vb = row_lerp(std::integral_constant<int, 0>{}, rb0, rb1, wbu, wbd);
                static_for<0, WS>([&](auto kc) TPIV_LAMBDA_INLINE {
                    constexpr int k = decltype(kc)::value;
                    if constexpr (k % 8 == 0 && k > 0) __builtin_amdgcn_sched_barrier(0);
                    if constexpr (LAZY && k % 16 == 0 && k > 0) pull(std::integral_constant<int, k / 16 + 1>{});
                    const float4 wx = wbuf[k];
                    const float na = row_lerp(std::integral_constant<int, k + 1>{}, ra0, ra1, wau, wad);
                    const float nb = row_lerp(std::integral_constant<int, k + 1>{}, rb0, rb1, wbu, wbd);
#ifdef TPIV_MUTANT_LERP
                    x[k].x = fmaf(na, wx.y * 1.001f, va * wx.x);
#else
                    x[k].x = fmaf(na, wx.y, va * wx.x);
#endif
                    x[k].y = fmaf(nb, wx.w, vb * wx.z);
                    va = na;
                    vb = nb;
                });
            } else {
            unsigned dmask_a = c.ydeg_a ? ~0u : 0u, dmask_b = c.ydeg_b ? ~0u : 0u;
            asm volatile("" : "+v"(dmask_a), "+v"(dmask_b));
            static_for<0, WS>([&](auto kc) TPIV_LAMBDA_INLINE {
                constexpr int k = decltype(kc)::value;
                if constexpr (k % 8 == 0 && k > 0) __builtin_amdgcn_sched_barrier(0);
                const float4 wx = wbuf[k];
                x[k].x = bilerp_ref_m(byte_f<k, NB>(ra0), byte_f<k + 1, NB>(ra0), byte_f<k, NB>(ra1),
                                      byte_f<k + 1, NB>(ra1), wx.x, wx.y, c.wya_up, c.wya_dn, dmask_a);
                x[k].y = bilerp_ref_m(byte_f<k, NB>(rb0), byte_f<k + 1, NB>(rb0), byte_f<k, NB>(rb1),
                                      byte_f<k + 1, NB>(rb1), wx.z, wx.w, c.wyb_up, c.wyb_dn, dmask_b);
            });
            }
            wave_sync();
        } else {
            wave_sync();
            static_for<0, RBH>([&](auto hc) TPIV_LAMBDA_INLINE {
            constexpr int k0 = decltype(hc)::value * RBL;
#pragma unroll UNR_CWS
            for (int k = 0; k < RBL; ++k) {
                const float nxa = (gx0f + (float)(k0 + k)) - vx;
                const float uxa_f = ceilf(nxa), dxa_f = floorf(nxa);
                const int uxa = f2i_sat_t(uxa_f), dxa = f2i_sat_t(dxa_f);
                rowbuf[k] = bilerp_ref(fetch_clamped_t(fa, (long long)c.dya * p.W + dxa, HW),
                                       fetch_clamped_t(fa, (long long)c.dya * p.W + uxa, HW),
                                       fetch_clamped_t(fa, (long long)c.uya * p.W + dxa, HW),
                                       fetch_clamped_t(fa, (long long)c.uya * p.W + uxa, HW), uxa_f - nxa,
                                       nxa - dxa_f, c.wya_up, c.wya_dn, c.ydeg_a || (uxa == dxa));
            }
#pragma unroll
            for (int k = 0; k < RBL; ++k) x[k0 + k].x = (FAST && TPIV_SDWA_LERP) ? rowbuf[k] * SDWA_DN : rowbuf[k];
#pragma unroll UNR_CWS
            for (int k = 0; k < RBL; ++k) {
                const float nxb = (gx0f + (float)(k0 + k)) + vx;
                const float uxb_f = ceilf(nxb), dxb_f = floorf(nxb);
                const int uxb = f2i_sat_t(uxb_f), dxb = f2i_sat_t(dxb_f);
                rowbuf[k] = bilerp_ref(fetch_clamped_t(fb, (long long)c.dyb * p.W + dxb, HW),
                                       fetch_clamped_t(fb, (long long)c.dyb * p.W + uxb, HW),
                                       fetch_clamped_t(fb, (long long)c.uyb * p.W + dxb, HW),
                                       fetch_clamped_t(fb, (long long)c.uyb * p.W + uxb, HW), uxb_f - nxb,
                                       nxb - dxb_f, c.wyb_up, c.wyb_dn, c.ydeg_b || (uxb == dxb));
            }
#pragma unroll
            for (int k = 0; k < RBL; ++k) x[k0 + k].y = (FAST && TPIV_SDWA_LERP) ? rowbuf[k] * SDWA_DN : rowbuf[k];
            });
            wave_sync();
        }
        sa = 0.f;
        sb = 0.f;
        if constexpr (!FAST) {
#pragma unroll
            for (int k = 0; k < WS; ++k) {
                sa += x[k].x;
                sb += x[k].y;
            }
        }
    }
}

template <int WS>
__device__ __forceinline__ unsigned long long exclusion_row_mask(int m, int ys, int wv) {
    static_assert(WS <= 64, "one 64-bit mask per row");
    const int my_ = m / WS, mx_ = m % WS, KD = WS * WS;
    const int dj = ys - my_;
    unsigned long long ex = 0ull;
    auto span = [&](int lo_, int hi_) TPIV_LAMBDA_INLINE {
        lo_ = lo_ < 0 ? 0 : lo_;
        hi_ = hi_ > WS - 1 ? WS - 1 : hi_;
        if (lo_ > hi_) return 0ull;
        const unsigned long long ones = (hi_ - lo_ + 1) >= 64 ? ~0ull : ((1ull << (hi_ - lo_ + 1)) - 1ull);
        return ones << lo_;
    };
    if (dj >= -wv && dj <= wv) ex |= span(mx_ - wv, mx_ + wv);
    if (dj + 1 >= -wv && dj + 1 <= wv) ex |= span(mx_ - wv + WS, mx_ + wv + WS);
    if (dj - 1 >= -wv && dj - 1 <= wv) ex |= span(mx_ - wv - WS, mx_ + wv - WS);
    if (ys == 0 && (m - wv - wv * WS) <= 0) ex |= 1ull;
    if (ys == WS - 1 && (m + wv + wv * WS) >= KD - 1) ex |= 1ull << (WS - 1);
    return ex;
}

__device__ __forceinline__ float max3_skip_nan(float a, float b, float c) {
    float o;
    asm("v_max3_f32 %0, %1, %2, %3" : "=v"(o) : "v"(a), "v"(b), "v"(c));
    return o;
}
__device__ __forceinline__ float max_skip_nan(float a, float b) {
    float o;
    asm("v_max_f32 %0, %1, %2" : "=v"(o) : "v"(a), "v"(b));
    return o;
}

template <int WS, bool PLANAR, bool SCALED = false>
__device__ __forceinline__ void peak_analysis(const PassParams& p, const float (&row)[WS], float* tile, int w, int r,
                                              bool active, bool dead, size_t fidx, float scale = 1.0f) {
    using G = TileGeo<WS, PLANAR>;
    constexpr bool SMALLMAP = G::WPW * WS * G::MAP_PITCH > G::LDS_FLOATS;
    static_assert(G::WPW * 3 * G::MAP_PITCH <= G::LDS_FLOATS, "map rows must fit the tile LDS");
    float* my_map = tile + w * ((SMALLMAP ? 3 : WS) * G::MAP_PITCH);
    const int ys = (r + WS / 2) % WS;
    float cmin = 3.4e38f, rraw = -3.4e38f;
#pragma unroll
    for (int k = 0; k < WS; ++k) {
        cmin = fminf(cmin, row[k]);
        rraw = fmaxf(rraw, row[k]);
    }
    cmin = grp_min<WS>(cmin);
    const float ncs = -(cmin * scale);
    auto shifted = [&](float c_) TPIV_LAMBDA_INLINE {
        if constexpr (SCALED) return __fadd_rn(fmaf(c_, scale, ncs), 1e-7f);
        else return __fadd_rn(__fsub_rn(c_, cmin), 1e-7f);
    };
    if constexpr (!SMALLMAP) {
        static_for<0, WS>([&](auto kc) TPIV_LAMBDA_INLINE {
            constexpr int xsft = decltype(kc)::value;
            my_map[ys * G::MAP_PITCH + xsft] = row[(xsft + WS / 2) % WS];
        });
    }
    const float rmax = shifted(rraw);
    const float gmax = grp_reduce<WS>(rmax, [](float a, float b) TPIV_LAMBDA_INLINE { return fmaxf(a, b); });
    auto imin = [](int a, int b) TPIV_LAMBDA_INLINE { return a < b ? a : b; };
    const int ywin = grp_reduce<WS>(rmax == gmax ? ys : WS - 1, imin);
    const int row0 = SMALLMAP ? ywin - 1 : 0;
    if constexpr (SMALLMAP) {
        wave_sync();
        const int slot = ys - row0;
        if (slot >= 0 && slot <= 2) {
            static_for<0, WS>([&](auto kc) TPIV_LAMBDA_INLINE {
                constexpr int xsft = decltype(kc)::value;
                my_map[slot * G::MAP_PITCH + xsft] = row[(xsft + WS / 2) % WS];
            });
        }
    }
    wave_sync();

    if (p.dbg_corr != nullptr && active) {
        int yy = ys;
        asm volatile("" : "+v"(yy));
        float* d = p.dbg_corr + fidx * WS * WS + yy * WS;
        static_for<0, WS>([&](auto kc) TPIV_LAMBDA_INLINE {
            constexpr int xsft = decltype(kc)::value;
            d[xsft] = shifted(row[(xsft + WS / 2) % WS]);
        });
    }
    const int xwin = grp_reduce<WS>(shifted(my_map[(ywin - row0) * G::MAP_PITCH + r]) == gmax ? r : WS - 1, imin);

    const int m = ywin * WS + xwin;
    const int KD = WS * WS;
    const int wv = p.val_win;
    float sraw;
    {
        const unsigned long long ex = exclusion_row_mask<WS>(m, ys, wv);
        const int exl = (int)(unsigned)ex, exh = (int)(unsigned)(ex >> 32);
        float acc = __int_as_float(-1);
        static_for<0, WS / 2>([&](auto kc) TPIV_LAMBDA_INLINE {
            constexpr int x0 = 2 * decltype(kc)::value, x1 = x0 + 1;
            const int k0 = __builtin_amdgcn_sbfe(x0 < 32 ? exl : exh, x0 & 31, 1);
            const int k1 = __builtin_amdgcn_sbfe(x1 < 32 ? exl : exh, x1 & 31, 1);
            const float v0 = __int_as_float(__float_as_int(row[(x0 + WS / 2) % WS]) | k0);
            const float v1 = __int_as_float(__float_as_int(row[(x1 + WS / 2) % WS]) | k1);
            acc = max3_skip_nan(acc, v0, v1);
        });
        sraw = acc;
    }
    sraw = grp_reduce<WS>(sraw, [](float a, float b) TPIV_LAMBDA_INLINE { return max_skip_nan(a, b); });
    const float second_v = sraw != sraw ? gmax : shifted(sraw);

    {
        int left = m + 1, right = m - 1, top = m + WS, bot = m - WS;
        if (left >= KD - 1) left = m;
        if (right <= 0) right = m;
        if (top >= KD - 1) top = m;
        if (bot <= 0) bot = m;
        int q = m;
        q = (r == 1) ? left : q;
        q = (r == 2) ? right : q;
        q = (r == 3) ? top : q;
        q = (r == 4) ? bot : q;
        float outv = shifted(my_map[(q / WS - row0) * G::MAP_PITCH + (q % WS)]);
        outv = (r == 5) ? second_v : outv;
        outv = (r == 6) ? __int_as_float(m) : outv;
        outv = (r == 7) ? __int_as_float(dead ? 1 : 0) : outv;
        if (r < 8 && active) p.peak_raw[fidx * 8 + r] = outv;
    }
}



template <int WS>
__device__ __forceinline__ void peak_candidates(const PassParams& p, const float (&row)[WS], float* tile, int w, int r,
                                                bool active, bool dead, size_t fidx, float band_abs) {
    static_assert(WS == 8 || WS == 16 || WS == 32 || WS == 64, "64 / WS windows per wavefront");
    auto wballot = [&](bool pred) TPIV_LAMBDA_INLINE {
        const unsigned long long b_ = __ballot(pred);
        if constexpr (WS == 64) return b_;
        else return (b_ >> (w * WS)) & ((1ull << WS) - 1ull);
    };
    auto any_left = [](unsigned long long mk) TPIV_LAMBDA_INLINE {
        if constexpr (WS == 64) return mk != 0ull;
        else return __ballot(mk != 0ull) != 0ull;
    };
    auto mine_left = [](unsigned long long mk) TPIV_LAMBDA_INLINE {
        if constexpr (WS == 64) return true;
        else return mk != 0ull;
    };
    float* const my_row = tile + w * WS;
    const int ys = (r + WS / 2) % WS;
    float rmin = 3.4e38f, rmax = -3.4e38f;
#pragma unroll
    for (int k = 0; k < WS; ++k) {
        rmin = fminf(rmin, row[k]);
        rmax = fmaxf(rmax, row[k]);
    }
    const float cmin = grp_min<WS>(rmin);
    const float gmax = grp_reduce<WS>(rmax, [](float a, float b) TPIV_LAMBDA_INLINE { return fmaxf(a, b); });
    const float band = fmaxf(p.exact_band_range * (gmax - cmin), band_abs);
    bool open = !(band > 0.0f) || !(gmax > cmin);
    auto park = [&](int rl) TPIV_LAMBDA_INLINE {
        wave_sync();
        if (r == rl) {
#pragma unroll
            for (int k = 0; k < WS; ++k) my_row[(k + WS / 2) % WS] = row[k];
        }
        wave_sync();
        return my_row[r];
    };
    auto row_of_lane = [](int rl) TPIV_LAMBDA_INLINE { return (rl + WS / 2) % WS; };
    int m = 0;
    {
        const unsigned long long rows = wballot(rmax >= gmax - band);
        open = open || __popcll(rows) != 1;
        const int rl = rows ? (int)__builtin_ctzll(rows) : 0;
        const unsigned long long cols = wballot(park(rl) >= gmax - band);
        open = open || __popcll(cols) != 1;
        m = row_of_lane(rl) * WS + (cols ? (int)__builtin_ctzll(cols) : 0);
    }
    const int wv = p.val_win;
    int s[EXACT_MAX_SECOND] = {-1, -1, -1};
    {
        const unsigned long long ex = exclusion_row_mask<WS>(m, ys, wv);
        const int exl = (int)(unsigned)ex, exh = (int)(unsigned)(ex >> 32);
        int smax = -1;
        static_for<0, WS>([&](auto kc) TPIV_LAMBDA_INLINE {
            constexpr int xsft = decltype(kc)::value;
            constexpr int xo = (xsft + WS / 2) % WS;
            const int kill = __builtin_amdgcn_sbfe(xsft < 32 ? exl : exh, xsft & 31, 1);
            const int cnd = __float_as_int(__fsub_rn(row[xo], cmin)) | kill;
            smax = cnd > smax ? cnd : smax;
        });
        const int sall = grp_reduce<WS>(smax, [](int a, int b) TPIV_LAMBDA_INLINE { return a > b ? a : b; });
        const float thr = __int_as_float(sall) - band;
        unsigned long long rows = sall >= 0 ? wballot(smax >= 0 && __int_as_float(smax) >= thr) : 0ull;
        open = open || __popcll(rows) > EXACT_MAX_SECOND;
        int ns = 0;
        for (int it = 0; it < EXACT_MAX_SECOND; ++it) {
            if (!any_left(rows)) break;
            const bool on = mine_left(rows);
            const int rl = on ? (int)__builtin_ctzll(rows) : 0;
            rows &= rows - 1;
            const int yr = row_of_lane(rl);
            const unsigned long long exr = exclusion_row_mask<WS>(m, yr, wv);
            unsigned long long cols = wballot(__fsub_rn(park(rl), cmin) >= thr) & ~exr;
            cols = on ? cols : 0ull;
            for (int k = 0; k < WS; ++k) {
                if (!any_left(cols)) break;
                const bool has = mine_left(cols);
                const int q = yr * WS + (has ? (int)__builtin_ctzll(cols) : 0);
                cols &= cols - 1;
                s[0] = (has && ns == 0) ? q : s[0];
                s[1] = (has && ns == 1) ? q : s[1];
                s[2] = (has && ns == 2) ? q : s[2];
                ns += has ? 1 : 0;
            }
        }
        open = open || ns > EXACT_MAX_SECOND;
    }
    int n[EXACT_MAX_MIN] = {-1, -1, -1, -1};
    {
        const float thr = cmin + band;
        unsigned long long rows = wballot(rmin <= thr);
        bool over = __popcll(rows) > EXACT_MAX_MIN;
        int nn = 0;
        for (int it = 0; it < EXACT_MAX_MIN; ++it) {
            if (!any_left(rows)) break;
            const bool on = mine_left(rows);
            const int rl = on ? (int)__builtin_ctzll(rows) : 0;
            rows &= rows - 1;
            const int yr = row_of_lane(rl);
            unsigned long long cols = wballot(park(rl) <= thr);
            cols = on ? cols : 0ull;
            over = over || nn + __popcll(cols) > EXACT_MAX_MIN;
            for (int k = 0; k < EXACT_MAX_MIN; ++k) {
                if (!any_left(cols)) break;
                const bool has = mine_left(cols) && cols != 0ull && nn < EXACT_MAX_MIN;
                const int q = yr * WS + (cols ? (int)__builtin_ctzll(cols) : 0);
                cols &= cols - 1;
                n[0] = (has && nn == 0) ? q : n[0];
                n[1] = (has && nn == 1) ? q : n[1];
                n[2] = (has && nn == 2) ? q : n[2];
                n[3] = (has && nn == 3) ? q : n[3];
                nn += has ? 1 : 0;
            }
        }
        n[3] = over ? -2 : n[3];
    }
    if (r == 0 && active) {
        const int m_out = dead ? -2 : (open ? -1 : m);
        auto pack = [](int lo_, int hi_) TPIV_LAMBDA_INLINE { return ((unsigned)lo_ & 0xffffu) | ((unsigned)hi_ << 16); };
        uint4 rec;
        rec.x = pack(m_out, s[0]);
        rec.y = pack(s[1], s[2]);
        rec.z = pack(n[0], n[1]);
        rec.w = pack(n[2], n[3]);
        p.cand[fidx] = rec;
    }
}

template <int WS, int MODE, int OCC, bool FAST, bool CAND, int ROLE = 0>
__device__ __forceinline__ void xcorr_tile_body(const PassParams& p) {
    constexpr bool PLANAR = OCC > 2;
    using G = TileGeo<WS, PLANAR>;
    static_assert(WS == 8 || WS == 16 || WS == 32 || WS == 64, "tile sizes of this kernel");
    constexpr int RBH = 64 * (WS + 1) <= G::LDS_FLOATS ? 1 : 2;
    static_assert(MODE == MODE_PASS1 || 64 * (WS / RBH + 1) <= G::LDS_FLOATS,
                  "slow-path row buffer (shifted passes) must fit the tile LDS");
    constexpr int LDSF = (MODE == MODE_CWS && CoopGeo<WS>::ON && CoopGeo<WS>::LDS_FLOATS > G::LDS_FLOATS)
                             ? CoopGeo<WS>::LDS_FLOATS : G::LDS_FLOATS;
    __shared__ __attribute__((aligned(16))) float tile[LDSF];

#ifndef TPIV_TWREG32
#define TPIV_TWREG32 0
#endif
    using TW = std::conditional_t<((WS == 32 && TPIV_TWREG32) || WS == 16), TwRegs<WS>, TwLiteral>;
    TW tw;
    if constexpr (!std::is_same<TW, TwLiteral>::value) tw.init();

    const int N = p.n_rows * p.n_cols;
    const int groups = (N + G::WPW - 1) / G::WPW;
    const bool listed = ROLE == 0 && MODE != MODE_PASS1 && p.list_mode != 0;
    const int items = listed ? __builtin_amdgcn_readfirstlane((int)*p.slow_count) : p.batch * groups;
    const int st = p.ws - p.ov;
    auto real_item = [&](int pos) TPIV_LAMBDA_INLINE { return listed ? __builtin_amdgcn_readfirstlane(p.slow_list[pos]) : pos; };

    constexpr int QCH = WS <= 16 ? 4 : 1;
    const int xcd = blockIdx.x & 7;
    const int chunk = (int)(((long long)items + 7) / 8);
    const int lo = __builtin_amdgcn_readfirstlane(xcd * chunk < items ? xcd * chunk : items);
    const int hi = __builtin_amdgcn_readfirstlane(items - lo > chunk ? lo + chunk : items);
    unsigned* const ctr = p.work_ctr + xcd * 16;
    int q_base = 0;
    int q_left = 0;
    auto q_issue = [&]() TPIV_LAMBDA_INLINE -> unsigned {
        unsigned v = 0;
        if (QCH == 1 || q_left == 0) {
            if (fresh_lane() == 0) v = atomicAdd(ctr, (unsigned)QCH);
        }
        return v;
    };
    auto q_take = [&](unsigned q_raw) TPIV_LAMBDA_INLINE -> int {
        if (QCH == 1 || q_left == 0) {
            const unsigned v = (unsigned)__builtin_amdgcn_readfirstlane((int)q_raw);
            q_base = v < (unsigned)(hi - lo) ? lo + (int)v : hi;
            q_left = QCH;
        }
        const int it = q_base + (QCH - q_left);
        --q_left;
        return it;
    };

    auto geom_of = [&](int pos, int w) TPIV_LAMBDA_INLINE {
        ItemGeom g;
        const int item = real_item(pos);
        g.pair = fast_div(item, p.groups_magic, p.groups_shift);
        const int gi = item - g.pair * groups;
        const int win_raw = gi * G::WPW + w;
        g.active = win_raw < N ? 1 : 0;
        g.win = g.active ? win_raw : N - 1;
        const int wrow = fast_div(g.win, p.ncols_magic, p.ncols_shift);
        g.y0 = wrow * st;
        g.x0 = (g.win - wrow * p.n_cols) * st;
        g.fidx = (size_t)g.pair * N + g.win;
        return g;
    };
    auto shift_of = [&](const ItemGeom& g, float& vx, float& vy) TPIV_LAMBDA_INLINE {
        if constexpr (MODE == MODE_PASS1) {
            vx = 0.f;
            vy = 0.f;
        } else {
            if constexpr (MODE == MODE_CWS) {
                pred_half_shift_cws_f32(p, g.fidx, vx, vy);
            } else {
                double sx, sy;
                pred_half_shift<MODE>(p, g.fidx, sx, sy);
                vx = (float)sx;
                vy = (float)sy;
            }
        }
    };

    int item = q_take(q_issue());
    if (item >= hi) return;
    int nitem = q_take(q_issue());
    constexpr bool RECOMPUTE = WS >= 32;
    float vx, vy;
    RawRows<WS, MODE> raw;
    ItemGeom gcur;
    CoopOff<WS> coff;
    if constexpr (MODE == MODE_CWS) coff.init(fresh_lane() % WS, p.W);
    {
        const int l0 = fresh_lane();
        gcur = geom_of(item, l0 / WS);
        shift_of(gcur, vx, vy);
        issue_rows<WS, MODE, FAST>(p, gcur, l0 % WS, vx, vy, raw, coff);
    }

    TPIV_STAMP_DECL
    TPIV_STAMP_START;
    for (int nnitem; item < hi; item = nitem, nitem = nnitem) {
        const unsigned q_raw = q_issue();
#ifdef TPIV_STAMPS
        ++st_iter;
#endif
        const int lane = fresh_lane();
        const int w = lane / WS;
        const int r = lane % WS;
        const ItemGeom g = RECOMPUTE ? geom_of(item, w) : gcur;
        const bool active = g.active != 0;
        const size_t fidx = g.fidx;
        const int nit = nitem < hi ? nitem : item;
        const ItemGeom gnext = geom_of(nit, w);
        float nvx, nvy;
        shift_of(gnext, nvx, nvy);

        if constexpr (ROLE == 1) {
            if (!raw.reg) {
                if (lane == 0) p.slow_list[atomicAdd(p.slow_count, 1u)] = item;
                nnitem = q_take(q_raw);
                issue_rows<WS, MODE, FAST>(p, gnext, r, nvx, nvy, raw, coff);
                vx = nvx;
                vy = nvy;
                if constexpr (!RECOMPUTE) gcur = gnext;
                continue;
            }
        }
        cf x[WS];
        float sa, sb;
        constexpr int NBS = WS >= 32 ? G::WPW : 1;
        int band_s[NBS];
        TPIV_STAMP(0);
        RowSquares sq;
        convert_rows<WS, MODE, RBH, FAST, CAND, ROLE == 1 ? 1 : 0>(p, g, r, lane, vx, vy, raw, x, sa, sb, tile, &sq);
        TPIV_STAMP(1);
        if constexpr (WS >= 64) nnitem = q_take(q_raw);
        if constexpr (WS <= 32) issue_rows<WS, MODE, FAST>(p, gnext, r, nvx, nvy, raw, coff);

        if (p.dbg_win != nullptr && active) {
            int rr = r;
            asm volatile("" : "+v"(rr));
            float* d = p.dbg_win + fidx * 2 * WS * WS + rr * WS;
            constexpr float UNS = (MODE == MODE_CWS && FAST && TPIV_SDWA_LERP) ? SDWA_INV : 1.0f;
#pragma unroll
            for (int k = 0; k < WS; ++k) {
                d[k] = x[k].x * UNS;
                d[WS * WS + k] = x[k].y * UNS;
            }
        }

        bool dead = false;
        float end_scale = 1.0f;
        constexpr bool FASTN = FAST && MODE != MODE_PASS1;
        if constexpr (!FASTN) {
            sa = grp_sum<WS>(sa);
            sb = grp_sum<WS>(sb);
            const float ma = sa * (1.0f / (WS * WS)), mb = sb * (1.0f / (WS * WS));
            float ka = 1.f, kb = 1.f;
            if constexpr (MODE == MODE_PASS1) {
                dead = (sa == 0.f) || (sb == 0.f);
                ka = dead ? 0.f : 1.0f / ma;
                kb = dead ? 0.f : 1.0f / mb;
            }
            if constexpr (CAND) {
                auto uadd = [](unsigned a_, unsigned b_) TPIV_LAMBDA_INLINE { return a_ + b_; };
                const unsigned saa = grp_reduce<WS>(sq.aa, uadd), sbb = grp_reduce<WS>(sq.bb, uadd);
                constexpr double NN = (double)(WS * WS);
                const double da = (double)sa, db = (double)sb;
                const float ea = (float)__fma_rn(-da, da, NN * (double)saa), eb = (float)__fma_rn(-db, db, NN * (double)sbb);
                const float e_plus = (0.5f / (float)(WS * WS)) * (ea * (ka * ka) + eb * (kb * kb));
                const float bnd = dead ? 0.f : p.exact_band * e_plus;
                if constexpr (WS >= 32) {
                    static_for<0, G::WPW>([&](auto wc) TPIV_LAMBDA_INLINE {
                        band_s[decltype(wc)::value] = __builtin_amdgcn_readlane(__float_as_int(bnd), decltype(wc)::value * WS);
                    });
                } else {
                    band_s[0] = __float_as_int(bnd);
                }
            }
            constexpr float PRE = 0.5f / (float)WS;
            const float oa = -ma * ka, ob = -mb * kb;
            const float kas = ka * PRE, kbs = kb * PRE, oas = oa * PRE, obs = ob * PRE;
#pragma unroll
            for (int k = 0; k < WS; ++k) {
                x[k].x = fmaf(x[k].x, kas, oas);
                x[k].y = fmaf(x[k].y, kbs, obs);
            }
        }

        TPIV_STAMP(2);
        fft_inreg<WS, 1>(x, tw);
        if constexpr (FASTN) {
            constexpr int P0 = FFT_POS<0, WS>;
            const float ta = grp_sum<WS>(x[P0].x);
            const float tb = grp_sum<WS>(x[P0].y);
            x[P0].x -= ta * (1.0f / WS);
            x[P0].y -= tb * (1.0f / WS);
            end_scale = 0.25f / (float)(WS * WS);
            if constexpr (MODE == MODE_CWS && TPIV_SDWA_LERP) end_scale *= SDWA_INV * SDWA_INV;
        }
        TPIV_STAMP(3);
        transpose_tile<WS, true, PLANAR>(x, tile, fresh_lane());
        TPIV_STAMP(4);
        fft_inreg<WS, 1>(x, tw);
        TPIV_STAMP(5);

        {
            const int lane_c = fresh_lane();
            const int r_c = lane_c % WS;
            const int partner = (lane_c - r_c) + ((WS - r_c) % WS);
            auto cross = [&](cf zk, cf zm) TPIV_LAMBDA_INLINE {
                const float a_ = zk.x, b_ = zk.y, c_ = zm.x, d_ = zm.y;
                cf pr;
                pr.x = (a_ * d_ + b_ * c_) * 2.0f;
                pr.y = (c_ * c_ - a_ * a_) + (d_ * d_ - b_ * b_);
                return pr;
            };
            static_for<0, WS / 2 + 1>([&](auto kc) TPIV_LAMBDA_INLINE {
                constexpr int ky = decltype(kc)::value;
                constexpr int nky = (WS - ky) % WS;
                constexpr int p1 = FFT_POS<ky, WS>, p2 = FFT_POS<nky, WS>;
                const cf z1 = x[p1];
                if constexpr (ky == nky) {
                    cf m1;
                    m1.x = __shfl(z1.x, partner, 64);
                    m1.y = __shfl(z1.y, partner, 64);
                    x[p1] = cross(z1, m1);
                } else {
                    const cf z2 = x[p2];
                    cf m1, m2;
                    m1.x = __shfl(z2.x, partner, 64);
                    m1.y = __shfl(z2.y, partner, 64);
                    m2.x = __shfl(z1.x, partner, 64);
                    m2.y = __shfl(z1.y, partner, 64);
                    x[p1] = cross(z1, m1);
                    x[p2] = cross(z2, m2);
                }
            });
        }

        TPIV_STAMP(6);
        cf t[WS];
        static_for<0, WS>([&](auto kc) TPIV_LAMBDA_INLINE {
            constexpr int ky = decltype(kc)::value;
            t[ky] = x[FFT_POS<ky, WS>];
        });
        fft_inreg<WS, -1>(t, tw);
        TPIV_STAMP(7);
#ifndef TPIV_C2R
#define TPIV_C2R 1
#endif
        float crow[WS];
#ifndef TPIV_C2R64
#define TPIV_C2R64 1
#endif
        if constexpr (TPIV_C2R && (WS <= 32 || (TPIV_C2R64 && WS == 64))) {
            cf hs[WS / 2 + 1], z[WS / 2];
            transpose_half<WS, PLANAR>(t, hs, tile, fresh_lane());
            TPIV_STAMP(8);
            c2r_inreg<WS>(hs, z);
            static_for<0, WS>([&](auto xc) TPIV_LAMBDA_INLINE {
                constexpr int x_ = decltype(xc)::value;
                crow[x_] = (x_ & 1) ? z[FFT_POS<x_ / 2, WS / 2>].y : z[FFT_POS<x_ / 2, WS / 2>].x;
            });
        } else {
            transpose_tile<WS, true, PLANAR>(t, tile, fresh_lane());
            TPIV_STAMP(8);
            fft_inreg<WS, -1>(t, tw);
            static_for<0, WS>([&](auto xc) TPIV_LAMBDA_INLINE {
                constexpr int x_ = decltype(xc)::value;
                crow[x_] = t[FFT_POS<x_, WS>].x;
            });
        }
        wave_sync();
        TPIV_STAMP(9);

        auto band_of = [&](int w_) TPIV_LAMBDA_INLINE {
            int b_ = band_s[0];
            static_for<1, NBS>([&](auto wc) TPIV_LAMBDA_INLINE { b_ = w_ == decltype(wc)::value ? band_s[decltype(wc)::value] : b_; });
            return __int_as_float(b_);
        };
        if constexpr (WS > 32) {
            const int lane_p = fresh_lane();
            issue_rows<WS, MODE, FAST>(p, geom_of(nit, lane_p / WS), lane_p % WS, nvx, nvy, raw, coff);
        }
        vx = nvx;
        vy = nvy;
        if constexpr (!RECOMPUTE) gcur = gnext;

        TPIV_STAMP(10);
        if constexpr (RECOMPUTE) {
            const int lane_e = fresh_lane();
            const int w_e = lane_e / WS, r_e = lane_e % WS;
            const int item_e = real_item(item);
            const int pair_e = fast_div(item_e, p.groups_magic, p.groups_shift);
            const int win_raw_e = (item_e - pair_e * groups) * G::WPW + w_e;
            const bool active_e = win_raw_e < N;
            const int win_e = active_e ? win_raw_e : N - 1;
            const size_t fidx_e = (size_t)pair_e * N + win_e;
            if constexpr (CAND) peak_candidates<WS>(p, crow, tile, w_e, r_e, active_e, dead, fidx_e, band_of(w_e));
            else peak_analysis<WS, PLANAR, FASTN>(p, crow, tile, w_e, r_e, active_e, dead, fidx_e, end_scale);
        } else {
            if constexpr (CAND) peak_candidates<WS>(p, crow, tile, w, r, active, dead, fidx, band_of(w));
            else peak_analysis<WS, PLANAR, FASTN>(p, crow, tile, w, r, active, dead, fidx, end_scale);
        }
        wave_sync();
        if constexpr (WS < 64) nnitem = q_take(q_raw);
        TPIV_STAMP(13);
    }
    TPIV_STAMP_FLUSH(p);
}

template <int WS, int MODE, int OCC, bool FAST>
__global__ __launch_bounds__(64, OCC) void xcorr_tile_kernel(PassParams p) {
    xcorr_tile_body<WS, MODE, OCC, FAST, false>(p);
}
template <int WS, int MODE>
__global__ __launch_bounds__(64, 3) void xcorr_tile_fastpath_kernel(PassParams p) {
    xcorr_tile_body<WS, MODE, 3, true, false, 1>(p);
}
template <int WS>
__global__ __launch_bounds__(64, tile_occ_c(WS, MODE_PASS1)) void xcorr_tile_cand_kernel(PassParams p) {
    xcorr_tile_body<WS, MODE_PASS1, tile_occ_c(WS, MODE_PASS1), true, true>(p);
}

template <int WS, bool PLANAR>
__global__ __launch_bounds__(64, 2) void peak_debug_kernel(PassParams p, const float* maps, int n_maps) {
    using G = TileGeo<WS, PLANAR>;
    __shared__ float tile[G::LDS_FLOATS];
    const int lane = threadIdx.x;
    const int w = lane / WS, r = lane % WS;
    const int win_raw = blockIdx.x * G::WPW + w;
    const bool active = win_raw < n_maps;
    const int win = active ? win_raw : n_maps - 1;
    float crow[WS];
    const int ys = (r + WS / 2) % WS;
#pragma unroll
    for (int xo = 0; xo < WS; ++xo) crow[xo] = maps[((size_t)win * WS + ys) * WS + (xo + WS / 2) % WS];
    peak_analysis<WS, PLANAR>(p, crow, tile, w, r, active, false, (size_t)win);
}

template <int WS>
hipError_t launch_peak_debug(const PassParams& p, const float* maps, int n_maps, int planar, hipStream_t stream) {
    using G = TileGeo<WS, false>;
    const int blocks = (n_maps + G::WPW - 1) / G::WPW;
    if (planar)
        hipLaunchKernelGGL((peak_debug_kernel<WS, true>), dim3(blocks), dim3(64), 0, stream, p, maps, n_maps);
    else
        hipLaunchKernelGGL((peak_debug_kernel<WS, false>), dim3(blocks), dim3(64), 0, stream, p, maps, n_maps);
    return hipGetLastError();
}

template <int WS, int MODE>
static hipError_t launch_tile(const PassParams& p_in, int n_cu, hipStream_t stream) {
    using G = TileGeo<WS>;
    PassParams p = p_in;
    const int N = p.n_rows * p.n_cols;
    const long long groups = (N + G::WPW - 1) / G::WPW;
    const long long items = (long long)p.batch * groups;
    if (items <= 0 || items >= (1ll << 31) - 64) return hipErrorInvalidValue;
    fast_div_setup((unsigned)groups, p.groups_magic, p.groups_shift);
    fast_div_setup((unsigned)p.n_cols, p.ncols_magic, p.ncols_shift);
    long long blocks = items;
    static const int wg_per_cu = [] {
        const char* e = getenv("TPIV_WG_PER_CU");
        return e ? atoi(e) : 0;
    }();
    const long long cap = (long long)n_cu * (wg_per_cu > 0 ? wg_per_cu : 64);
    if (blocks > cap) blocks = cap;
    blocks = (blocks + 7) / 8 * 8;
    constexpr int OCC = tile_occ_c(WS, MODE);
    if constexpr (MODE != MODE_PASS1) {
        if (p.precision != 0) {
            hipLaunchKernelGGL((xcorr_tile_kernel<WS, MODE, OCC, false>), dim3((unsigned)blocks), dim3(64), 0, stream, p);
            return hipGetLastError();
        }
    }
#ifdef TPIV_EXPERIMENT
    static const int occ_env = [] {
        const char* e = getenv("TPIV_OCC");
        return e ? atoi(e) : 0;
    }();
    if (occ_env == 2 && OCC != 2) {
        hipLaunchKernelGGL((xcorr_tile_kernel<WS, MODE, 2, true>), dim3((unsigned)blocks), dim3(64), 0, stream, p);
        return hipGetLastError();
    }
    if constexpr (WS <= 32 || MODE != MODE_CWS) {
        if (occ_env == 3 && OCC != 3) {
            hipLaunchKernelGGL((xcorr_tile_kernel<WS, MODE, 3, true>), dim3((unsigned)blocks), dim3(64), 0, stream, p);
            return hipGetLastError();
        }
    }
    if constexpr (WS <= 32) {
        if (occ_env == 4 && OCC != 4) {
            hipLaunchKernelGGL((xcorr_tile_kernel<WS, MODE, 4, true>), dim3((unsigned)blocks), dim3(64), 0, stream, p);
            return hipGetLastError();
        }
    }
#endif
    if constexpr (tile_split64(WS, MODE)) {
        if (p.slow_list != nullptr && p.slow_count != nullptr) {
            hipLaunchKernelGGL((xcorr_tile_fastpath_kernel<WS, MODE>), dim3((unsigned)blocks), dim3(64), 0, stream, p);
            hipError_t e_ = hipGetLastError();
            if (e_ != hipSuccess) return e_;
            e_ = hipMemsetAsync(p.work_ctr, 0, TILE_CTR_BYTES, stream);
            if (e_ != hipSuccess) return e_;
            PassParams q = p;
            q.list_mode = 1;
            long long blocks2 = (long long)n_cu * 8;
            if (blocks2 > blocks) blocks2 = blocks;
            blocks2 = (blocks2 + 7) / 8 * 8;
            hipLaunchKernelGGL((xcorr_tile_kernel<WS, MODE, OCC, true>), dim3((unsigned)blocks2), dim3(64), 0, stream, q);
            return hipGetLastError();
        }
    }
    hipLaunchKernelGGL((xcorr_tile_kernel<WS, MODE, OCC, true>), dim3((unsigned)blocks), dim3(64), 0, stream, p);
    return hipGetLastError();
}

template <int WS>
hipError_t launch_xcorr_tile_cand_ws(const PassParams& p_in, int n_cu, hipStream_t stream) {
    using G = TileGeo<WS>;
    PassParams p = p_in;
    const int N = p.n_rows * p.n_cols;
    const long long groups = (N + G::WPW - 1) / G::WPW;
    const long long items = (long long)p.batch * groups;
    if (items <= 0 || items >= (1ll << 31) - 64 || p.cand == nullptr) return hipErrorInvalidValue;
    fast_div_setup((unsigned)groups, p.groups_magic, p.groups_shift);
    fast_div_setup((unsigned)p.n_cols, p.ncols_magic, p.ncols_shift);
    long long blocks = items < (long long)n_cu * 64 ? items : (long long)n_cu * 64;
    blocks = (blocks + 7) / 8 * 8;
    hipLaunchKernelGGL((xcorr_tile_cand_kernel<WS>), dim3((unsigned)blocks), dim3(64), 0, stream, p);
    return hipGetLastError();
}

template <int WS>
hipError_t launch_xcorr_tile_ws(const PassParams& p, int mode, int n_cu, hipStream_t stream) {
    switch (mode) {
        case MODE_PASS1: return launch_tile<WS, MODE_PASS1>(p, n_cu, stream);
        case MODE_DWS: return launch_tile<WS, MODE_DWS>(p, n_cu, stream);
        case MODE_CWS: return launch_tile<WS, MODE_CWS>(p, n_cu, stream);
        default: return hipErrorInvalidValue;
    }
}

}
```

Before: 16480.

## Add optional fold of exact refine into ws64 tile kernel and restructure refine launch

Moves exact-refine helpers into a shared header and adds a compile-time option to run the exact integer refinement for 64x64 windows inside the CWS tile kernel, reusing the tile LDS and skipping the separate refine launch. The option is off by default. On the default path, peak_candidates now parks the first minimum row alongside the maximum row, and the standalone refine kernel is re-templated on wave count with a default of two waves per block. The fold trades an extra kernel launch and re-read of window data for more registers and LDS pressure in the tile kernel.

```diff
diff --git a/torchpiv_amd/csrc/exact_cells.hpp b/torchpiv_amd/csrc/exact_cells.hpp
--- /dev/null
+++ b/torchpiv_amd/csrc/exact_cells.hpp
@@ -0,0 +1,250 @@
+#pragma once
+#include <hip/hip_runtime.h>
+#include <stdint.h>
+
+#include "piv_kernels.h"
+
+namespace tpiv {
+
+template <int W>
+struct XGeo {
+    static constexpr int NDW = W / 4;
+    static constexpr int XP = 2 * NDW + 1;
+    static constexpr int GROUP = W < 64 ? W : 64;
+    static constexpr int WPW = 64 / GROUP;
+    static constexpr int PARTS = W / GROUP;
+    static constexpr int WAVES = W == 128 ? 2 : 4;
+    static constexpr int WINS = WAVES * WPW / PARTS;
+    static constexpr int KD = W * W;
+    static constexpr bool COOP = W >= 32;
+    static constexpr int P16 = W / 16;
+    static constexpr int LW = GROUP * PARTS;
+    static constexpr int AP = NDW + 4;
+    static_assert(!COOP || (W * AP <= W * XP && (LW * P16) == W * P16), "the hand-over tile lives in the parked rows' memory");
+};
+constexpr int XCELLS = 5 + EXACT_MAX_SECOND + EXACT_MAX_MIN;
+
+#if defined(__HIP_DEVICE_COMPILE__)
+template <int OFF>
+__device__ __forceinline__ uint32_t lds_rd32(unsigned addr) {
+    uint32_t v;
+    asm volatile("ds_read_b32 %0, %1 offset:%2" : "=v"(v) : "v"(addr), "n"(OFF) : "memory");
+    return v;
+}
+__device__ __forceinline__ void lds_landed() { asm volatile("s_waitcnt lgkmcnt(0)" ::: "memory"); }
+__device__ __forceinline__ void lds_tie(uint32_t& v) { asm volatile("" : "+v"(v)); }
+#else
+template <int OFF>
+__host__ __device__ inline uint32_t lds_rd32(unsigned) { return 0u; }
+__host__ __device__ inline void lds_landed() {}
+__host__ __device__ inline void lds_tie(uint32_t&) {}
+#endif
+template <int N>
+__device__ __forceinline__ void read_span(const uint32_t* src, uint32_t (&w)[N]) {
+    const unsigned addr = (unsigned)(uintptr_t)src;
+    static_for<0, N>([&](auto ic) TPIV_LAMBDA_INLINE { w[decltype(ic)::value] = lds_rd32<4 * decltype(ic)::value>(addr); });
+    lds_landed();
+    static_for<0, N>([&](auto ic) TPIV_LAMBDA_INLINE { lds_tie(w[decltype(ic)::value]); });
+}
+
+__device__ __forceinline__ void list_append(const PassParams& p, bool want, long long it) {
+    const unsigned long long mk = __ballot(want);
+    if (mk == 0ull) return;
+    const int lane = (int)__builtin_amdgcn_mbcnt_hi(~0u, __builtin_amdgcn_mbcnt_lo(~0u, 0u));
+    const int leader = (int)__builtin_ctzll(mk);
+    unsigned base = 0u;
+    if (lane == leader) base = atomicAdd(p.fb_count, (unsigned)__popcll(mk));
+    base = (unsigned)__builtin_amdgcn_readlane((int)base, leader);
+    const unsigned rank = __builtin_amdgcn_mbcnt_hi((unsigned)(mk >> 32), __builtin_amdgcn_mbcnt_lo((unsigned)mk, 0u));
+    if (want) p.fb_list[base + rank] = (int)it;
+}
+
+__device__ __forceinline__ void exact_settle_early(const PassParams& p, int m, int r0, bool writer, double* out, long long it) {
+    list_append(p, m == -1 && r0 == 0 && writer, it);
+    if (m == -2 && r0 < 8 && writer) out[r0] = r0 == 6 ? 0.0 : 1.0;
+}
+
+template <int W>
+__device__ __forceinline__ int exact_cell_of(const uint4& rec, int m, int r0) {
+    constexpr int KD = W * W;
+    auto lo16 = [](unsigned v) TPIV_LAMBDA_INLINE { return (int)(short)(v & 0xffffu); };
+    auto hi16 = [](unsigned v) TPIV_LAMBDA_INLINE { return (int)(short)(v >> 16); };
+    int left = m + 1, right = m - 1, top = m + W, bot = m - W;
+    if (left >= KD - 1) left = m;
+    if (right <= 0) right = m;
+    if (top >= KD - 1) top = m;
+    if (bot <= 0) bot = m;
+    int q = -1;
+    q = r0 == 0 ? m : q;
+    q = r0 == 1 ? left : q;
+    q = r0 == 2 ? right : q;
+    q = r0 == 3 ? top : q;
+    q = r0 == 4 ? bot : q;
+    q = r0 == 5 ? hi16(rec.x) : q;
+    q = r0 == 6 ? lo16(rec.y) : q;
+    q = r0 == 7 ? hi16(rec.y) : q;
+    q = r0 == 8 ? lo16(rec.z) : q;
+    q = r0 == 9 ? hi16(rec.z) : q;
+    q = r0 == 10 ? lo16(rec.w) : q;
+    q = r0 == 11 ? hi16(rec.w) : q;
+    return q;
+}
+
+template <int W>
+__device__ __forceinline__ void exact_load_chunks(const PassParams& p, size_t off0, int tw, uint32_t (&ca)[XGeo<W>::P16][4],
+                                                  uint32_t (&cb)[XGeo<W>::P16][4]) {
+    using G = XGeo<W>;
+#pragma unroll
+    for (int k = 0; k < G::P16; ++k) {
+        const int ci = tw + G::LW * k, j = ci / G::P16, pt = ci % G::P16;
+        const size_t o_ = off0 + (size_t)j * p.W + 16 * pt;
+        load_dwords<4>(p.A + o_, ca[k]);
+        load_dwords<4>(p.B + o_, cb[k]);
+    }
+}
+
+template <int W, bool SUMS, typename SYNC>
+__device__ __forceinline__ void exact_stage_chunks(const uint32_t (&ca)[XGeo<W>::P16][4], const uint32_t (&cb)[XGeo<W>::P16][4],
+                                                   uint32_t* rows_b, int tw, int row, uint32_t (&a)[XGeo<W>::NDW],
+                                                   unsigned (&P)[16], SYNC lds_sync) {
+    using G = XGeo<W>;
+    constexpr int NDW = G::NDW, XP = G::XP;
+    uint4* const ta = reinterpret_cast<uint4*>(rows_b);
+#pragma unroll
+    for (int k = 0; k < G::P16; ++k) {
+        const int ci = tw + G::LW * k, j = ci / G::P16, pt = ci % G::P16;
+        ta[j * (G::AP / 4) + pt] = make_uint4(ca[k][0], ca[k][1], ca[k][2], ca[k][3]);
+    }
+    lds_sync();
+#pragma unroll
+    for (int k = 0; k < NDW / 4; ++k) {
+        const uint4 t = ta[row * (G::AP / 4) + k];
+        a[4 * k] = t.x, a[4 * k + 1] = t.y, a[4 * k + 2] = t.z, a[4 * k + 3] = t.w;
+    }
+    lds_sync();
+#pragma unroll
+    for (int k = 0; k < G::P16; ++k) {
+        const int ci = tw + G::LW * k, j = ci / G::P16, pt = ci % G::P16;
+#pragma unroll
+        for (int c = 0; c < 4; ++c) {
+            if constexpr (SUMS) P[13] = __builtin_amdgcn_sad_u8(cb[k][c], 0u, P[13]);
+            rows_b[j * XP + 4 * pt + c] = cb[k][c];
+            rows_b[j * XP + NDW + 4 * pt + c] = cb[k][c];
+        }
+    }
+    if constexpr (SUMS) {
+#pragma unroll
+        for (int i = 0; i < NDW; ++i) P[12] = __builtin_amdgcn_sad_u8(a[i], 0u, P[12]);
+    }
+}
+
+template <int W>
+__device__ __forceinline__ void exact_eval_cells(int q, int g, int row, const uint32_t (&a)[XGeo<W>::NDW], const uint32_t* rows_b,
+                                                 unsigned (&P)[16]) {
+    using G = XGeo<W>;
+    constexpr int NDW = G::NDW, XP = G::XP;
+    static_for<0, XCELLS>([&](auto cc) TPIV_LAMBDA_INLINE {
+        constexpr int c = decltype(cc)::value;
+        int qc = __builtin_amdgcn_readlane(q, c);
+        bool any = qc >= 0;
+        static_for<1, G::WPW>([&](auto wc) TPIV_LAMBDA_INLINE {
+            constexpr int k = decltype(wc)::value;
+            const int qk = __builtin_amdgcn_readlane(q, k * G::GROUP + c);
+            any = any || qk >= 0;
+            qc = g == k ? qk : qc;
+        });
+        if (any) {
+            const bool on = qc >= 0;
+            const int qq = on ? qc : 0;
+            const int dy = qq / W - W / 2, dx = qq % W - W / 2;
+            const int brow = (row + dy) & (W - 1), bx = dx & (W - 1);
+            const uint32_t* src = rows_b + brow * XP + (bx >> 2);
+            const unsigned sh = (unsigned)(bx & 3);
+            uint32_t w[NDW + 1];
+            read_span<NDW + 1>(src, w);
+            unsigned acc = 0;
+#pragma unroll
+            for (int i = 0; i < NDW; ++i) acc = __builtin_amdgcn_udot4(a[i], __builtin_amdgcn_alignbyte(w[i + 1], w[i], sh), acc, false);
+            P[c] = on ? acc : 0u;
+        }
+    });
+}
+
+template <int GROUP>
+__device__ __forceinline__ void exact_reduce(const unsigned (&P)[16], int lane, unsigned (&T)[4]) {
+    const bool odd = lane & 1, hi = lane & 2;
+    unsigned Q[8];
+#pragma unroll
+    for (int j = 0; j < 8; ++j) {
+        const unsigned keep = odd ? P[2 * j + 1] : P[2 * j], send = odd ? P[2 * j] : P[2 * j + 1];
+        Q[j] = keep + (unsigned)dpp_i<DPP_XOR1>((int)send);
+    }
+#pragma unroll
+    for (int j = 0; j < 4; ++j) {
+        const unsigned keep = hi ? Q[2 * j + 1] : Q[2 * j], send = hi ? Q[2 * j] : Q[2 * j + 1];
+        unsigned t = keep + (unsigned)dpp_i<DPP_XOR2>((int)send);
+        t += (unsigned)dpp_i<0x128>((int)t);
+        t += (unsigned)dpp_i<0x124>((int)t);
+        if constexpr (GROUP >= 32) {
+            auto r = __builtin_amdgcn_permlane16_swap(t, t, false, false);
+            t = r[0] + r[1];
+        }
+        if constexpr (GROUP >= 64) {
+            auto r = __builtin_amdgcn_permlane32_swap(t, t, false, false);
+            t = r[0] + r[1];
+        }
+        T[j] = t;
+    }
+}
+
+__device__ __forceinline__ void decide_and_store(const PassParams& p, const uint4& rec, int r0, bool go, bool writer, bool have,
+                                                 int m, unsigned S, unsigned sa, unsigned sb, double kd, double* out, long long it) {
+    auto hi16 = [](unsigned v) TPIV_LAMBDA_INLINE { return (int)(short)(v >> 16); };
+    auto umin = [](unsigned x, unsigned y) TPIV_LAMBDA_INLINE { return x < y ? x : y; };
+    auto umax = [](unsigned x, unsigned y) TPIV_LAMBDA_INLINE { return x > y ? x : y; };
+    auto uadd = [](unsigned x, unsigned y) TPIV_LAMBDA_INLINE { return x + y; };
+    constexpr int S0 = 5, N0 = 5 + EXACT_MAX_SECOND;
+    S = r0 < XCELLS ? S : 0u;
+    const unsigned s_min = grp_reduce<16>((have && r0 >= N0 && r0 < XCELLS) ? S : 0xffffffffu, umin);
+    const unsigned s_low = grp_reduce<16>((have && r0 < XCELLS) ? S : 0xffffffffu, umin);
+    const unsigned s_top = grp_reduce<16>((have && r0 < N0) ? S : 0u, umax);
+    const unsigned s_m = grp_reduce<16>(r0 == 0 ? S : 0u, umax);
+    const unsigned s_second = grp_reduce<16>((have && r0 >= S0 && r0 < N0) ? S : 0u, umax);
+    const unsigned n_second = grp_reduce<16>((have && r0 >= S0 && r0 < N0) ? 1u : 0u, uadd);
+    const bool min_overflow = hi16(rec.w) == -2;
+    const bool redo = s_top > s_m || s_low < s_min || s_min == 0xffffffffu || sa == 0u || sb == 0u ||
+                      (min_overflow && s_min != 0u);
+    list_append(p, go && redo && r0 == 0 && writer, it);
+    const double scale = (kd * kd) / ((double)sa * (double)sb);
+    const unsigned mine = r0 == 5 ? s_second : S;
+    double v = __fma_rn((double)(mine - s_min), scale, 1e-7);
+    v = (r0 == 5 && n_second == 0u) ? 0.0 : v;
+    v = r0 == 6 ? (double)m : v;
+    v = r0 == 7 ? 0.0 : v;
+    if (go && !redo && r0 < 8 && writer) out[r0] = v;
+}
+
+__device__ __forceinline__ void exact_window64(const PassParams& p, const uint4& rec, const uint32_t (&ca)[XGeo<64>::P16][4],
+                                               const uint32_t (&cb)[XGeo<64>::P16][4], uint32_t* rows_b, int lane,
+                                               unsigned sa, unsigned sb, long long it) {
+    constexpr int W = 64;
+    auto lo16 = [](unsigned v) TPIV_LAMBDA_INLINE { return (int)(short)(v & 0xffffu); };
+    const int m = lo16(rec.x);
+    double* const out = reinterpret_cast<double*>(p.peak_raw) + (size_t)it * 8;
+    exact_settle_early(p, m, lane, true, out, it);
+    if (m < 0) return;
+    const int q = exact_cell_of<W>(rec, m, lane);
+    unsigned P[16];
+#pragma unroll
+    for (int k = 0; k < 16; ++k) P[k] = 0u;
+    uint32_t a[XGeo<W>::NDW];
+    exact_stage_chunks<W, false>(ca, cb, rows_b, lane, lane, a, P, [] { wave_sync(); });
+    wave_sync();
+    exact_eval_cells<W>(q, 0, lane, a, rows_b, P);
+    unsigned T[4];
+    exact_reduce<64>(P, lane, T);
+    const unsigned S = lane < 4 ? T[0] : (lane < 8 ? T[1] : T[2]);
+    decide_and_store(p, rec, lane, true, true, q >= 0, m, S, sa, sb, (double)(W * W), out, it);
+}
+
+}
diff --git a/torchpiv_amd/csrc/piv_kernels.h b/torchpiv_amd/csrc/piv_kernels.h
--- a/torchpiv_amd/csrc/piv_kernels.h
+++ b/torchpiv_amd/csrc/piv_kernels.h
@@ -117,6 +117,10 @@
 #define TPIV_SPLIT64 1
 #endif
 constexpr bool tile_split64(int ws, int mode) { return TPIV_SPLIT64 && ws == 64 && mode == MODE_CWS; }
+#ifndef TPIV_FOLD_REFINE64
+#define TPIV_FOLD_REFINE64 0
+#endif
+constexpr bool exact_fold64(int ws) { return TPIV_FOLD_REFINE64 && ws == 64; }
 #ifndef TPIV_OCC64C
 #define TPIV_OCC64C 2
 #endif
diff --git a/torchpiv_amd/csrc/piv_launch.hip b/torchpiv_amd/csrc/piv_launch.hip
--- a/torchpiv_amd/csrc/piv_launch.hip
+++ b/torchpiv_amd/csrc/piv_launch.hip
@@ -272,8 +272,10 @@
         }
         if (e != hipSuccess) return e;
         mark(0);
-        e = launch_exact_refine(p, n_cu, stream);
-        if (e != hipSuccess) return e;
+        if (!exact_fold64(p.ws)) {
+            e = launch_exact_refine(p, n_cu, stream);
+            if (e != hipSuccess) return e;
+        }
         mark(1);
         if (tile_size(p.ws) || p.ws == 128) {
             e = launch_xcorr_f64_list(p, n_cu, stream);
diff --git a/torchpiv_amd/csrc/xcorr_exact.hip b/torchpiv_amd/csrc/xcorr_exact.hip
--- a/torchpiv_amd/csrc/xcorr_exact.hip
+++ b/torchpiv_amd/csrc/xcorr_exact.hip
@@ -9,90 +9,10 @@
 namespace {
 
 template <int W>
-struct XGeo {
-    static constexpr int NDW = W / 4;
-    static constexpr int XP = 2 * NDW + 1;
-    static constexpr int GROUP = W < 64 ? W : 64;
-    static constexpr int WPW = 64 / GROUP;
-    static constexpr int PARTS = W / GROUP;
-    static constexpr int WAVES = W == 128 ? 2 : 4;
-    static constexpr int WINS = WAVES * WPW / PARTS;
-    static constexpr int KD = W * W;
-    static constexpr bool COOP = W >= 32;
-    static constexpr int P16 = W / 16;
-    static constexpr int LW = GROUP * PARTS;
-    static constexpr int AP = NDW + 4;
-    static_assert(!COOP || (W * AP <= W * XP && (LW * P16) == W * P16), "the hand-over tile lives in the parked rows' memory");
-};
-constexpr int XCELLS = 5 + EXACT_MAX_SECOND + EXACT_MAX_MIN;
-
-#if defined(__HIP_DEVICE_COMPILE__)
-template <int OFF>
-__device__ __forceinline__ uint32_t lds_rd32(unsigned addr) {
-    uint32_t v;
-    asm volatile("ds_read_b32 %0, %1 offset:%2" : "=v"(v) : "v"(addr), "n"(OFF) : "memory");
-    return v;
-}
-__device__ __forceinline__ void lds_landed() { asm volatile("s_waitcnt lgkmcnt(0)" ::: "memory"); }
-__device__ __forceinline__ void lds_tie(uint32_t& v) { asm volatile("" : "+v"(v)); }
-#else
-template <int OFF>
-__host__ __device__ inline uint32_t lds_rd32(unsigned) { return 0u; }
-__host__ __device__ inline void lds_landed() {}
-__host__ __device__ inline void lds_tie(uint32_t&) {}
-#endif
-template <int N>
-__device__ __forceinline__ void read_span(const uint32_t* src, uint32_t (&w)[N]) {
-    const unsigned addr = (unsigned)(uintptr_t)src;
-    static_for<0, N>([&](auto ic) TPIV_LAMBDA_INLINE { w[decltype(ic)::value] = lds_rd32<4 * decltype(ic)::value>(addr); });
-    lds_landed();
-    static_for<0, N>([&](auto ic) TPIV_LAMBDA_INLINE { lds_tie(w[decltype(ic)::value]); });
-}
-
-__device__ __forceinline__ void list_append(const PassParams& p, bool want, long long it) {
-    const unsigned long long mk = __ballot(want);
-    if (mk == 0ull) return;
-    const int lane = (int)__builtin_amdgcn_mbcnt_hi(~0u, __builtin_amdgcn_mbcnt_lo(~0u, 0u));
-    const int leader = (int)__builtin_ctzll(mk);
-    unsigned base = 0u;
-    if (lane == leader) base = atomicAdd(p.fb_count, (unsigned)__popcll(mk));
-    base = (unsigned)__builtin_amdgcn_readlane((int)base, leader);
-    if (want) p.fb_list[base + (unsigned)__popcll(mk & ((1ull << lane) - 1ull))] = (int)it;
-}
-
-__device__ __forceinline__ void decide_and_store(const PassParams& p, const uint4& rec, int r0, bool go, bool writer, bool have,
-                                                 int m, unsigned S, unsigned sa, unsigned sb, double kd, double* out, long long it) {
-    auto hi16 = [](unsigned v) TPIV_LAMBDA_INLINE { return (int)(short)(v >> 16); };
-    auto umin = [](unsigned x, unsigned y) TPIV_LAMBDA_INLINE { return x < y ? x : y; };
-    auto umax = [](unsigned x, unsigned y) TPIV_LAMBDA_INLINE { return x > y ? x : y; };
-    auto uadd = [](unsigned x, unsigned y) TPIV_LAMBDA_INLINE { return x + y; };
-    constexpr int S0 = 5, N0 = 5 + EXACT_MAX_SECOND;
-    S = r0 < XCELLS ? S : 0u;
-    const unsigned s_min = grp_reduce<16>((have && r0 >= N0 && r0 < XCELLS) ? S : 0xffffffffu, umin);
-    const unsigned s_low = grp_reduce<16>((have && r0 < XCELLS) ? S : 0xffffffffu, umin);
-    const unsigned s_top = grp_reduce<16>((have && r0 < N0) ? S : 0u, umax);
-    const unsigned s_m = grp_reduce<16>(r0 == 0 ? S : 0u, umax);
-    const unsigned s_second = grp_reduce<16>((have && r0 >= S0 && r0 < N0) ? S : 0u, umax);
-    const unsigned n_second = grp_reduce<16>((have && r0 >= S0 && r0 < N0) ? 1u : 0u, uadd);
-    const bool min_overflow = hi16(rec.w) == -2;
-    const bool redo = s_top > s_m || s_low < s_min || s_min == 0xffffffffu || sa == 0u || sb == 0u ||
-                      (min_overflow && s_min != 0u);
-    list_append(p, go && redo && r0 == 0 && writer, it);
-    const double scale = (kd * kd) / ((double)sa * (double)sb);
-    const unsigned mine = r0 == 5 ? s_second : S;
-    double v = __fma_rn((double)(mine - s_min), scale, 1e-7);
-    v = (r0 == 5 && n_second == 0u) ? 0.0 : v;
-    v = r0 == 6 ? (double)m : v;
-    v = r0 == 7 ? 0.0 : v;
-    if (go && !redo && r0 < 8 && writer) out[r0] = v;
-}
-
-template <int W>
-__global__ __launch_bounds__(64 * XGeo<W>::WAVES) void xcorr_exact_refine_kernel(PassParams p) {
+__device__ __forceinline__ void refine_window(const PassParams& p, uint32_t (*parked)[W * XGeo<W>::XP],
+                                              unsigned (&joined)[2][16], long long first) {
     using G = XGeo<W>;
     constexpr int NDW = G::NDW, XP = G::XP, KD = G::KD;
-    __shared__ __attribute__((aligned(16))) uint32_t parked[G::WINS][W * XP];
-    __shared__ unsigned joined[2][16];
     const int wave = __builtin_amdgcn_readfirstlane((int)(threadIdx.x >> 6));
     const int lane = (int)(threadIdx.x & 63);
     const int g = lane / G::GROUP, r0 = lane % G::GROUP;
@@ -102,9 +22,9 @@
     uint32_t* const rows_b = parked[wslot];
     const int N = p.n_rows * p.n_cols;
     const long long total = (long long)p.batch * N;
-    const int xcd = blockIdx.x & 7, slot = blockIdx.x >> 3;
-    const long long chunk = (total + 7) / 8;
-    const long long in_chunk = (long long)slot * G::WINS + wslot;
+    const int xcd = blockIdx.x & 7;
+    const long long chunk = (total + 7) / 8;
+    const long long in_chunk = first + wslot;
     const long long it_raw = (long long)xcd * chunk + in_chunk;
     const bool valid = in_chunk < chunk && it_raw < total;
     const long long it = valid ? it_raw : 0;
@@ -117,13 +37,7 @@
     uint32_t ca[G::COOP ? G::P16 : 1][4], cb[G::COOP ? G::P16 : 1][4];
     const int tw = r0 + 64 * part;
     if constexpr (G::COOP) {
-#pragma unroll
-        for (int k = 0; k < G::P16; ++k) {
-            const int ci = tw + G::LW * k, j = ci / G::P16, pt = ci % G::P16;
-            const size_t o_ = off0 + (size_t)j * p.W + 16 * pt;
-            load_dwords<4>(p.A + o_, ca[k]);
-            load_dwords<4>(p.B + o_, cb[k]);
-        }
+        exact_load_chunks<W>(p, off0, tw, ca, cb);
     } else {
         const size_t off = off0 + (size_t)row * p.W;
         load_dwords<NDW>(p.A + off, a);
@@ -131,35 +45,14 @@
     }
     const uint4 rec = p.cand[it];
     auto lo16 = [](unsigned v) TPIV_LAMBDA_INLINE { return (int)(short)(v & 0xffffu); };
-    auto hi16 = [](unsigned v) TPIV_LAMBDA_INLINE { return (int)(short)(v >> 16); };
     const int m = valid ? lo16(rec.x) : -3;
     double* const out = reinterpret_cast<double*>(p.peak_raw) + (size_t)it * 8;
     const bool writer = part == 0;
-    list_append(p, m == -1 && r0 == 0 && writer, it);
-    if (m == -2 && r0 < 8 && writer) out[r0] = r0 == 6 ? 0.0 : 1.0;
+    exact_settle_early(p, m, r0, writer, out, it);
     const bool go = m >= 0;
     if (__ballot(go) == 0ull) return;
 
-    int q = -1;
-    if (go) {
-        int left = m + 1, right = m - 1, top = m + W, bot = m - W;
-        if (left >= KD - 1) left = m;
-        if (right <= 0) right = m;
-        if (top >= KD - 1) top = m;
-        if (bot <= 0) bot = m;
-        q = r0 == 0 ? m : q;
-        q = r0 == 1 ? left : q;
-        q = r0 == 2 ? right : q;
-        q = r0 == 3 ? top : q;
-        q = r0 == 4 ? bot : q;
-        q = r0 == 5 ? hi16(rec.x) : q;
-        q = r0 == 6 ? lo16(rec.y) : q;
-        q = r0 == 7 ? hi16(rec.y) : q;
-        q = r0 == 8 ? lo16(rec.z) : q;
-        q = r0 == 9 ? hi16(rec.z) : q;
-        q = r0 == 10 ? lo16(rec.w) : q;
-        q = r0 == 11 ? hi16(rec.w) : q;
-    }
+    const int q = go ? exact_cell_of<W>(rec, m, r0) : -1;
 
     unsigned P[16];
 #pragma unroll
@@ -169,31 +62,7 @@
         else wave_sync();
     };
     if constexpr (G::COOP) {
-        uint4* const ta = reinterpret_cast<uint4*>(rows_b);
-#pragma unroll
-        for (int k = 0; k < G::P16; ++k) {
-            const int ci = tw + G::LW * k, j = ci / G::P16, pt = ci % G::P16;
-            ta[j * (G::AP / 4) + pt] = make_uint4(ca[k][0], ca[k][1], ca[k][2], ca[k][3]);
-        }
-        lds_sync();
-#pragma unroll
-        for (int k = 0; k < NDW / 4; ++k) {
-            const uint4 t = ta[row * (G::AP / 4) + k];
-            a[4 * k] = t.x, a[4 * k + 1] = t.y, a[4 * k + 2] = t.z, a[4 * k + 3] = t.w;
-        }
-        lds_sync();
-#pragma unroll
-        for (int k = 0; k < G::P16; ++k) {
-            const int ci = tw + G::LW * k, j = ci / G::P16, pt = ci % G::P16;
-#pragma unroll
-            for (int c = 0; c < 4; ++c) {
-                P[13] = __builtin_amdgcn_sad_u8(cb[k][c], 0u, P[13]);
-                rows_b[j * XP + 4 * pt + c] = cb[k][c];
-                rows_b[j * XP + NDW + 4 * pt + c] = cb[k][c];
-            }
-        }
-#pragma unroll
-        for (int i = 0; i < NDW; ++i) P[12] = __builtin_amdgcn_sad_u8(a[i], 0u, P[12]);
+        exact_stage_chunks<W, true>(ca, cb, rows_b, tw, row, a, P, lds_sync);
     } else {
 #pragma unroll
         for (int i = 0; i < NDW; ++i) {
@@ -205,57 +74,9 @@
     }
     lds_sync();
 
-    static_for<0, XCELLS>([&](auto cc) TPIV_LAMBDA_INLINE {
-        constexpr int c = decltype(cc)::value;
-        int qc = __builtin_amdgcn_readlane(q, c);
-        bool any = qc >= 0;
-        static_for<1, G::WPW>([&](auto wc) TPIV_LAMBDA_INLINE {
-            constexpr int k = decltype(wc)::value;
-            const int qk = __builtin_amdgcn_readlane(q, k * G::GROUP + c);
-            any = any || qk >= 0;
-            qc = g == k ? qk : qc;
-        });
-        if (any) {
-            const bool on = qc >= 0;
-            const int qq = on ? qc : 0;
-            const int dy = qq / W - W / 2, dx = qq % W - W / 2;
-            const int brow = (row + dy) & (W - 1), bx = dx & (W - 1);
-            const uint32_t* src = rows_b + brow * XP + (bx >> 2);
-            const unsigned sh = (unsigned)(bx & 3);
-            uint32_t w[NDW + 1];
-            read_span<NDW + 1>(src, w);
-            unsigned acc = 0;
-#pragma unroll
-            for (int i = 0; i < NDW; ++i) acc = __builtin_amdgcn_udot4(a[i], __builtin_amdgcn_alignbyte(w[i + 1], w[i], sh), acc, false);
-            P[c] = on ? acc : 0u;
-        }
-    });
+    exact_eval_cells<W>(q, g, row, a, rows_b, P);
     unsigned T[4];
-    {
-        const bool odd = lane & 1, hi = lane & 2;
-        unsigned Q[8];
-#pragma unroll
-        for (int j = 0; j < 8; ++j) {
-            const unsigned keep = odd ? P[2 * j + 1] : P[2 * j], send = odd ? P[2 * j] : P[2 * j + 1];
-            Q[j] = keep + (unsigned)dpp_i<DPP_XOR1>((int)send);
-        }
-#pragma unroll
-        for (int j = 0; j < 4; ++j) {
-            const unsigned keep = hi ? Q[2 * j + 1] : Q[2 * j], send = hi ? Q[2 * j] : Q[2 * j + 1];
-            unsigned t = keep + (unsigned)dpp_i<DPP_XOR2>((int)send);
-            t += (unsigned)dpp_i<0x128>((int)t);
-            t += (unsigned)dpp_i<0x124>((int)t);
-            if constexpr (G::GROUP >= 32) {
-                auto r = __builtin_amdgcn_permlane16_swap(t, t, false, false);
-                t = r[0] + r[1];
-            }
-            if constexpr (G::GROUP >= 64) {
-                auto r = __builtin_amdgcn_permlane32_swap(t, t, false, false);
-                t = r[0] + r[1];
-            }
-            T[j] = t;
-        }
-    }
+    exact_reduce<G::GROUP>(P, lane, T);
     unsigned S = r0 < 4 ? T[0] : (r0 < 8 ? T[1] : (r0 < 12 ? T[2] : T[3]));
     if constexpr (G::PARTS == 2) {
         if (lane < 16) joined[wave][lane] = S;
@@ -275,6 +96,16 @@
     S = r0 < XCELLS ? S : 0u;
 
     decide_and_store(p, rec, r0, go, writer, q >= 0, m, S, sa, sb, (double)KD, out, it);
+}
+
+template <int W, int WV>
+__global__ __launch_bounds__(64 * WV) void xcorr_exact_refine_kernel(PassParams p) {
+    using G = XGeo<W>;
+    static_assert(G::PARTS == 1 || WV == 2, "128x128 windows take one workgroup of two wavefronts");
+    constexpr int WINS = WV * G::WPW / G::PARTS;
+    __shared__ __attribute__((aligned(16))) uint32_t parked[WINS][W * G::XP];
+    __shared__ unsigned joined[2][16];
+    refine_window<W>(p, parked, joined, (long long)(blockIdx.x >> 3) * WINS);
 }
 
 template <int W>
@@ -558,8 +389,21 @@
     using G = XGeo<W>;
     const long long total = (long long)p.batch * p.n_rows * p.n_cols;
     const long long chunk = (total + 7) / 8;
-    const long long slots = (chunk + G::WINS - 1) / G::WINS;
-    hipLaunchKernelGGL((xcorr_exact_refine_kernel<W>), dim3((unsigned)(slots * 8)), dim3(64 * G::WAVES), 0, stream, p);
+    static const int wv_env = [] { const char* e = getenv("TPIV_REFINE_WAVES"); return e ? atoi(e) : 0; }();
+    const int WV = G::PARTS == 2 ? 2 : (wv_env == 3 || wv_env == 4 ? wv_env : 2);
+    const long long wins = (long long)WV * G::WPW / G::PARTS;
+    const dim3 grid((unsigned)((chunk + wins - 1) / wins * 8)), block(64 * WV);
+    if constexpr (G::PARTS == 1) {
+        if (WV == 3) {
+            hipLaunchKernelGGL((xcorr_exact_refine_kernel<W, 3>), grid, block, 0, stream, p);
+            return hipGetLastError();
+        }
+        if (WV == 4) {
+            hipLaunchKernelGGL((xcorr_exact_refine_kernel<W, 4>), grid, block, 0, stream, p);
+            return hipGetLastError();
+        }
+    }
+    hipLaunchKernelGGL((xcorr_exact_refine_kernel<W, 2>), grid, block, 0, stream, p);
     return hipGetLastError();
 }
 
diff --git a/torchpiv_amd/csrc/xcorr_tile.hpp b/torchpiv_amd/csrc/xcorr_tile.hpp
--- a/torchpiv_amd/csrc/xcorr_tile.hpp
+++ b/torchpiv_amd/csrc/xcorr_tile.hpp
@@ -1108,9 +1108,13 @@
 
 
 
-template <int WS>
-__device__ __forceinline__ void peak_candidates(const PassParams& p, const float (&row)[WS], float* tile, int w, int r,
-                                                bool active, bool dead, size_t fidx, float band_abs) {
+}
+#include "exact_cells.hpp"
+namespace tpiv {
+
+template <int WS, bool STORE = true>
+__device__ __forceinline__ uint4 peak_candidates(const PassParams& p, const float (&row)[WS], float* tile, int w, int r,
+                                                 bool active, bool dead, size_t fidx, float band_abs) {
     static_assert(WS == 8 || WS == 16 || WS == 32 || WS == 64, "64 / WS windows per wavefront");
     auto wballot = [&](bool pred) TPIV_LAMBDA_INLINE {
         const unsigned long long b_ = __ballot(pred);
@@ -1147,12 +1151,26 @@
         return my_row[r];
     };
     auto row_of_lane = [](int rl) TPIV_LAMBDA_INLINE { return (rl + WS / 2) % WS; };
+    const float thr_min = cmin + band;
+    const unsigned long long rows_min = wballot(rmin <= thr_min);
+    float min_row0;
     int m = 0;
     {
         const unsigned long long rows = wballot(rmax >= gmax - band);
         open = open || __popcll(rows) != 1;
         const int rl = rows ? (int)__builtin_ctzll(rows) : 0;
-        const unsigned long long cols = wballot(park(rl) >= gmax - band);
+        const int rn = rows_min ? (int)__builtin_ctzll(rows_min) : 0;
+        float* const min_row = tile + 64 + w * WS;
+        wave_sync();
+        if (r == rl || r == rn) {
+            float* const dst = r == rl ? my_row : min_row;
+#pragma unroll
+            for (int k = 0; k < WS; ++k) dst[(k + WS / 2) % WS] = row[k];
+        }
+        wave_sync();
+        const float v_max = my_row[r];
+        min_row0 = rn == rl ? v_max : min_row[r];
+        const unsigned long long cols = wballot(v_max >= gmax - band);
         open = open || __popcll(cols) != 1;
         m = row_of_lane(rl) * WS + (cols ? (int)__builtin_ctzll(cols) : 0);
     }
@@ -1198,8 +1216,8 @@
     }
     int n[EXACT_MAX_MIN] = {-1, -1, -1, -1};
     {
-        const float thr = cmin + band;
-        unsigned long long rows = wballot(rmin <= thr);
+        const float thr = thr_min;
+        unsigned long long rows = rows_min;
         bool over = __popcll(rows) > EXACT_MAX_MIN;
         int nn = 0;
         for (int it = 0; it < EXACT_MAX_MIN; ++it) {
@@ -1208,7 +1226,7 @@
             const int rl = on ? (int)__builtin_ctzll(rows) : 0;
             rows &= rows - 1;
             const int yr = row_of_lane(rl);
-            unsigned long long cols = wballot(park(rl) <= thr);
+            unsigned long long cols = wballot((it == 0 ? min_row0 : park(rl)) <= thr);
             cols = on ? cols : 0ull;
             over = over || nn + __popcll(cols) > EXACT_MAX_MIN;
             for (int k = 0; k < EXACT_MAX_MIN; ++k) {
@@ -1225,16 +1243,15 @@
         }
         n[3] = over ? -2 : n[3];
     }
-    if (r == 0 && active) {
-        const int m_out = dead ? -2 : (open ? -1 : m);
-        auto pack = [](int lo_, int hi_) TPIV_LAMBDA_INLINE { return ((unsigned)lo_ & 0xffffu) | ((unsigned)hi_ << 16); };
-        uint4 rec;
-        rec.x = pack(m_out, s[0]);
-        rec.y = pack(s[1], s[2]);
-        rec.z = pack(n[0], n[1]);
-        rec.w = pack(n[2], n[3]);
-        p.cand[fidx] = rec;
-    }
+    const int m_out = dead ? -2 : (open ? -1 : m);
+    auto pack = [](int lo_, int hi_) TPIV_LAMBDA_INLINE { return ((unsigned)lo_ & 0xffffu) | ((unsigned)hi_ << 16); };
+    uint4 rec;
+    rec.x = pack(m_out, s[0]);
+    rec.y = pack(s[1], s[2]);
+    rec.z = pack(n[0], n[1]);
+    rec.w = pack(n[2], n[3]);
+    if (STORE && r == 0 && active) p.cand[fidx] = rec;
+    return rec;
 }
 
 template <int WS, int MODE, int OCC, bool FAST, bool CAND, int ROLE = 0>
@@ -1242,6 +1259,8 @@
     constexpr bool PLANAR = OCC > 2;
     using G = TileGeo<WS, PLANAR>;
     static_assert(WS == 8 || WS == 16 || WS == 32 || WS == 64, "tile sizes of this kernel");
+    constexpr bool FOLD = CAND && WS == 64 && TPIV_FOLD_REFINE64;
+    static_assert(!FOLD || 64 * XGeo<64>::XP <= G::LDS_FLOATS, "the fold parks frame b (64 x 33 dwords) in the tile");
     constexpr int RBH = 64 * (WS + 1) <= G::LDS_FLOATS ? 1 : 2;
     static_assert(MODE == MODE_PASS1 || 64 * (WS / RBH + 1) <= G::LDS_FLOATS,
                   "slow-path row buffer (shifted passes) must fit the tile LDS");
@@ -1368,6 +1387,7 @@
         float sa, sb;
         constexpr int NBS = WS >= 32 ? G::WPW : 1;
         int band_s[NBS];
+        int sum_a_s = 0, sum_b_s = 0;
         TPIV_STAMP(0);
         RowSquares sq;
         convert_rows<WS, MODE, RBH, FAST, CAND, ROLE == 1 ? 1 : 0>(p, g, r, lane, vx, vy, raw, x, sa, sb, tile, &sq);
@@ -1408,6 +1428,10 @@
                 const float ea = (float)__fma_rn(-da, da, NN * (double)saa), eb = (float)__fma_rn(-db, db, NN * (double)sbb);
                 const float e_plus = (0.5f / (float)(WS * WS)) * (ea * (ka * ka) + eb * (kb * kb));
                 const float bnd = dead ? 0.f : p.exact_band * e_plus;
+                if constexpr (FOLD) {
+                    sum_a_s = __builtin_amdgcn_readfirstlane((int)(unsigned)sa);
+                    sum_b_s = __builtin_amdgcn_readfirstlane((int)(unsigned)sb);
+                }
                 if constexpr (WS >= 32) {
                     static_for<0, G::WPW>([&](auto wc) TPIV_LAMBDA_INLINE {
                         band_s[decltype(wc)::value] = __builtin_amdgcn_readlane(__float_as_int(bnd), decltype(wc)::value * WS);
@@ -1518,6 +1542,11 @@
             static_for<1, NBS>([&](auto wc) TPIV_LAMBDA_INLINE { b_ = w_ == decltype(wc)::value ? band_s[decltype(wc)::value] : b_; });
             return __int_as_float(b_);
         };
+        uint32_t fca[FOLD ? XGeo<64>::P16 : 1][4], fcb[FOLD ? XGeo<64>::P16 : 1][4];
+        if constexpr (FOLD) {
+            const ItemGeom gf = geom_of(item, 0);
+            exact_load_chunks<64>(p, (size_t)gf.pair * p.H * p.W + (size_t)gf.y0 * p.W + gf.x0, fresh_lane(), fca, fcb);
+        }
         if constexpr (WS > 32) {
             const int lane_p = fresh_lane();
             issue_rows<WS, MODE, FAST>(p, geom_of(nit, lane_p / WS), lane_p % WS, nvx, nvy, raw, coff);
@@ -1536,8 +1565,18 @@
             const bool active_e = win_raw_e < N;
             const int win_e = active_e ? win_raw_e : N - 1;
             const size_t fidx_e = (size_t)pair_e * N + win_e;
-            if constexpr (CAND) peak_candidates<WS>(p, crow, tile, w_e, r_e, active_e, dead, fidx_e, band_of(w_e));
-            else peak_analysis<WS, PLANAR, FASTN>(p, crow, tile, w_e, r_e, active_e, dead, fidx_e, end_scale);
+            if constexpr (FOLD) {
+                const uint4 rec = peak_candidates<WS, false>(p, crow, tile, w_e, r_e, active_e, dead, fidx_e, band_of(w_e));
+                if (active_e) {
+                    wave_sync();
+                    exact_window64(p, rec, fca, fcb, reinterpret_cast<uint32_t*>(tile), lane_e, (unsigned)sum_a_s,
+                                   (unsigned)sum_b_s, (long long)fidx_e);
+                }
+            } else if constexpr (CAND) {
+                peak_candidates<WS>(p, crow, tile, w_e, r_e, active_e, dead, fidx_e, band_of(w_e));
+            } else {
+                peak_analysis<WS, PLANAR, FASTN>(p, crow, tile, w_e, r_e, active_e, dead, fidx_e, end_scale);
+            }
         } else {
             if constexpr (CAND) peak_candidates<WS>(p, crow, tile, w, r, active, dead, fidx, band_of(w));
             else peak_analysis<WS, PLANAR, FASTN>(p, crow, tile, w, r, active, dead, fidx, end_scale);
```

Measured after the change: 16750, median of 6. +1.6%, better.
